# ivpml84079/Probabilistic-Self-Update-Line-Vector-Set-Based-Point-Cloud-Registration

Hardware: NVIDIA B200
Metric: registrations/s (higher is better)
Workload: dtype f64+f32

## Files before the change

probabilistic-self-update-line-vector-set-based-point-cloud-registration_b200/csrc/capi.cu:

```cuda
#include <cuda_runtime.h>

#include <cmath>
#include <cstring>
#include <new>
#include <string>
#include <vector>

#include "common.cuh"
#include "engine.cuh"

namespace psulvsb {

static thread_local std::string g_last_error;

void set_error(const std::string& msg) { g_last_error = msg; }
int fail(int code, const std::string& msg) {
  g_last_error = msg;
  return code;
}

int sm_count() {
  static int cached[64];
  int dev = 0;
  if (cudaGetDevice(&dev) != cudaSuccess || dev < 0 || dev >= 64) return 148;
// ... 18 lines not shown
  }
  return PSULVSB_OK;
}

namespace {

template <typename T>
struct DeviceJob {
  T* d = nullptr;
  cudaStream_t st;
  explicit DeviceJob(cudaStream_t s) : st(s) {}
  int put(const T& h) {
    PSU_CUDA(cudaMallocAsync((void**)&d, sizeof(T), st));
    PSU_CUDA(cudaMemcpyAsync(d, &h, sizeof(T), cudaMemcpyHostToDevice, st));
    return PSULVSB_OK;
  }
  ~DeviceJob() {
    if (d) cudaFreeAsync(d, st);
  }
};

}
}

using namespace psulvsb;

struct psulvsb_handle_s {
  EnginePool* pool;
  Comm* comm;
  int device;
};

extern "C" {

int psulvsb_version(void) { return PSULVSB_VERSION; }

const char* psulvsb_last_error(void) { return g_last_error.c_str(); }

void psulvsb_default_params(psulvsb_params_t* p) {
  if (!p) return;
  std::memset(p, 0, sizeof(*p));
  p->noise_bound = 0.01;
  p->cbar2 = 1;
  p->estimate_scaling = 1;
  p->rotation_max_iterations = 100;
  p->rotation_gnc_factor = 1.4;
  p->rotation_cost_threshold = 1e-6;
  p->inlier_selection_mode = 0;
  p->kcore_heuristic_threshold = 0.5;
  p->score_noise_bound = 0.01;
  p->inloop_noise_bound = 0.05;
  p->inloop_cbar2 = 1;
  p->inloop_max_iterations = 100;
  p->inloop_gnc_factor = 1.4;
  p->inloop_cost_threshold = 0.005;
  p->rotation_similar = 0.01;
  p->local_max_iter = 10;
  p->tpro_host = 0.99;
  p->tpro_local = 0.99;
  p->host_round_limit = 5;
  p->wallclock_cap_s = 60.0;
  p->self_update = 1;
  p->seed = 0;
}

int psulvsb_device_count(void) {
  int n = 0;
  if (cudaGetDeviceCount(&n) != cudaSuccess) {
    cudaGetLastError();
    return 0;
  }
  return n;
}

int psulvsb_create(psulvsb_handle_t* out, int device) {
  if (!out) return fail(PSULVSB_ERR_INVALID, "psulvsb_create: out is NULL");
  *out = nullptr;
  if (int rc = need_device()) return rc;
  psulvsb_handle_s* h = new (std::nothrow) psulvsb_handle_s();
  if (!h) return fail(PSULVSB_ERR_INTERNAL, "out of host memory");
  h->comm = nullptr;
  h->device = device;
  const int rc = pool_create(&h->pool, device);
  if (rc) {
    delete h;
    return rc;
  }
  *out = h;
  return PSULVSB_OK;
}

int psulvsb_destroy(psulvsb_handle_t h) {
  if (!h) return PSULVSB_OK;
  comm_destroy(h->comm);
  pool_destroy(h->pool);
  delete h;
  return PSULVSB_OK;
}

int psulvsb_solve(psulvsb_handle_t h, const psulvsb_params_t* params, const psulvsb_problem_t* problem,
                  psulvsb_solution_t* solution, psulvsb_trace_t* trace) {
  if (!h || !params || !problem || !solution) return fail(PSULVSB_ERR_INVALID, "psulvsb_solve: NULL argument");
  return pool_solve_one(h->pool, params, problem, solution, trace);
}

int psulvsb_solve_batch(psulvsb_handle_t h, const psulvsb_params_t* params, const psulvsb_problem_t* problems, int B,
                        const uint64_t* seeds, psulvsb_solution_t* solutions) {
  if (!h || !params || !problems || !solutions || B <= 0)
    return fail(PSULVSB_ERR_INVALID, "psulvsb_solve_batch: NULL argument or B <= 0");
  return pool_solve_batch(h->pool, params, problems, B, seeds, solutions);
}

int psulvsb_batch_submit(psulvsb_handle_t h, const psulvsb_params_t* params, const psulvsb_problem_t* problems, int B,
                         const uint64_t* seeds, psulvsb_solution_t* solutions, uint64_t* ticket) {
  if (!h || !params || !problems || !solutions || !ticket || B <= 0)
    return fail(PSULVSB_ERR_INVALID, "psulvsb_batch_submit: NULL argument or B <= 0");
  return pool_submit(h->pool, params, problems, B, seeds, solutions, ticket);
}

int psulvsb_batch_wait(psulvsb_handle_t h, uint64_t ticket) {
  if (!h) return fail(PSULVSB_ERR_INVALID, "psulvsb_batch_wait: NULL handle");
  return pool_wait(h->pool, ticket);
}

int psulvsb_batch_upload(psulvsb_handle_t h, const psulvsb_problem_t* problems, int B) {
  if (!h || !problems || B <= 0) return fail(PSULVSB_ERR_INVALID, "psulvsb_batch_upload: NULL argument or B <= 0");
  return pool_upload(h->pool, problems, B);
}

int psulvsb_batch_solve_resident(psulvsb_handle_t h, const psulvsb_params_t* params, const uint64_t* seeds,
                                 psulvsb_solution_t* solutions, int n_solutions) {
  if (!h || !params || !solutions) return fail(PSULVSB_ERR_INVALID, "psulvsb_batch_solve_resident: NULL argument");
  const int B = pool_batch_size(h->pool);
  if (B <= 0) return fail(PSULVSB_ERR_INVALID, "psulvsb_batch_solve_resident: nothing is resident (upload first)");
  if (n_solutions != B)
    return fail(PSULVSB_ERR_INVALID, "psulvsb_batch_solve_resident: " + std::to_string(n_solutions) +
                                         " solution slots for a resident batch of " + std::to_string(B));
  return pool_solve_resident(h->pool, params, seeds, solutions, nullptr);
}

int psulvsb_debug_set(const char* name, double value) {
  if (!name) return fail(PSULVSB_ERR_INVALID, "psulvsb_debug_set: NULL name");
  DebugKnobs& k = debug_knobs();
  const std::string n(name);
  if (n == "gnc_deep_margin") k.gnc_deep_margin = value;
  else if (n == "gnc_prefetch") k.gnc_prefetch = (int)value;
  else if (n == "gnc_cluster") k.gnc_cluster = (int)value;
  else if (n == "gnc_park_pct") k.gnc_park_pct = (int)value;
  else if (n == "gnc_cps") k.gnc_cps = (int)value;
  else if (n == "gnc_grid_lv") k.gnc_grid_lv = (int)value;
  else if (n == "sample_list_cap_test") k.sample_list_cap_test = (int)value;
  else if (n == "k1_variant") k.k1_variant = (int)value;
  else if (n == "upload_prof") k.upload_prof = (int)value;
  else if (n == "reset") k = DebugKnobs();
  else return fail(PSULVSB_ERR_INVALID, "psulvsb_debug_set: unknown switch " + n);
  return PSULVSB_OK;
}

int psulvsb_batch_resident_size(psulvsb_handle_t h) { return h ? pool_batch_size(h->pool) : 0; }

int psulvsb_set_batching(psulvsb_handle_t h, int chunk, int lanes) {
  if (!h) return fail(PSULVSB_ERR_INVALID, "psulvsb_set_batching: NULL handle");
  return pool_set_batching(h->pool, chunk, lanes);
}

int psulvsb_set_host_threads(psulvsb_handle_t h, int n) {
  if (!h) return fail(PSULVSB_ERR_INVALID, "psulvsb_set_host_threads: NULL handle");
  return pool_set_host_threads(h->pool, n);
}

long long psulvsb_launch_count(psulvsb_handle_t h) { return h ? pool_launch_count(h->pool) : 0; }
double psulvsb_last_device_ms(psulvsb_handle_t h) { return h ? pool_last_device_ms(h->pool) : 0.0; }
double psulvsb_last_stage_ms(psulvsb_handle_t h, int which) { return h ? pool_last_stage_ms(h->pool, which) : 0.0; }
int psulvsb_last_ticks(psulvsb_handle_t h) { return h ? pool_last_ticks(h->pool) : 0; }
int psulvsb_last_chunk_ticks(psulvsb_handle_t h, int* out, int cap) {
  if (!h || (cap > 0 && !out)) return 0;
  return pool_last_chunk_ticks(h->pool, out, cap);
}


int psulvsb_pack_points(void* stream, const double* d_pts, int n, const double center[3], void* d_out_float4) {
  if (int rc = need_device()) return rc;
  if (!d_pts || !d_out_float4 || n < 0) return fail(PSULVSB_ERR_INVALID, "psulvsb_pack_points: bad argument");
  return launch_pack_points((cudaStream_t)stream, d_pts, n, center, (float4*)d_out_float4);
}

int psulvsb_consistency_mask_rows(void* stream, const void* d_src_f4, const void* d_dst_f4, const double* d_src64,
                                  const double* d_dst64, int n, int row_begin, int row_end, double beta,
                                  double coord_bound, uint32_t* d_mask, int row_stride_words, uint32_t* d_row_counts,
                                  unsigned long long* d_border_count) {
  if (int rc = need_device()) return rc;
  if (!d_src_f4 || !d_dst_f4 || !d_src64 || !d_dst64 || !d_mask)
    return fail(PSULVSB_ERR_INVALID, "psulvsb_consistency_mask: NULL array");
  if (n < 1 || row_begin < 0 || row_end > n || row_begin > row_end)
    return fail(PSULVSB_ERR_INVALID, "psulvsb_consistency_mask: bad n / row range");
  if (row_stride_words < (n + 31) / 32)
    return fail(PSULVSB_ERR_CAPACITY, "psulvsb_consistency_mask: row_stride_words < ceil(n / 32)");
  if (!(beta >= 0.0) || !(coord_bound >= 0.0) || !std::isfinite(beta) || !std::isfinite(coord_bound))
    return fail(PSULVSB_ERR_INVALID, "psulvsb_consistency_mask: beta / coord_bound must be finite and >= 0");
  if (((uintptr_t)d_src_f4 & 15) || ((uintptr_t)d_dst_f4 & 15))
    return fail(PSULVSB_ERR_INVALID, "psulvsb_consistency_mask: float4 arrays must be 16-byte aligned");
  if (row_begin == row_end) return PSULVSB_OK;
  cudaStream_t st = (cudaStream_t)stream;
  float4* il = nullptr;
  const size_t nrec = il_records((size_t)n);
  PSU_CUDA(cudaMallocAsync((void**)&il, sizeof(float4) * 2 * nrec, st));
  struct IlFree {
    float4* p;
    cudaStream_t s;
    ~IlFree() { cudaFreeAsync(p, s); }
  } il_free{il, st};
  if (int rc = launch_interleave_points(st, (const float4*)d_src_f4, n, il)) return rc;
  if (int rc = launch_interleave_points(st, (const float4*)d_dst_f4, n, il + nrec)) return rc;
  K1Job j;
  std::memset(&j, 0, sizeof(j));
  j.src = il;
  j.dst = il + nrec;
  j.src64 = d_src64;
  j.dst64 = d_dst64;
  j.n = n;
  j.row_begin = row_begin;
  j.row_end = row_end;
  j.c = make_k1_consts(beta, coord_bound);
  j.mask = d_mask;
  j.stride = row_stride_words;
  j.row_counts = d_row_counts;
  j.border = d_border_count;
  j.active = 1;
  if (d_row_counts) PSU_CUDA(cudaMemsetAsync(d_row_counts + row_begin, 0, sizeof(uint32_t) * (size_t)(row_end - row_begin), st));
  PSU_CUDA(cudaMemsetAsync(d_mask + (size_t)row_begin * row_stride_words, 0,
                           sizeof(uint32_t) * (size_t)(row_end - row_begin) * row_stride_words, st));
  DeviceJob<K1Job> dj(st);
  if (int rc = dj.put(j)) return rc;
  return launch_consistency_mask(st, dj.d, 1, n, row_end - row_begin, (row_stride_words & 7) == 0);
}

int psulvsb_consistency_mask(void* stream, const void* d_src_f4, const void* d_dst_f4, const double* d_src64,
                             const double* d_dst64, int n, double beta, double coord_bound, uint32_t* d_mask,
                             int row_stride_words, uint32_t* d_row_counts, unsigned long long* d_border_count) {
  return psulvsb_consistency_mask_rows(stream, d_src_f4, d_dst_f4, d_src64, d_dst64, n, 0, n, beta, coord_bound, d_mask,
                                       row_stride_words, d_row_counts, d_border_count);
}

int psulvsb_mask_symmetrize(void* stream, uint32_t* d_mask, int n, int row_stride_words) {
  if (int rc = need_device()) return rc;
  if (!d_mask || n < 1 || row_stride_words < (n + 31) / 32)
    return fail(PSULVSB_ERR_INVALID, "psulvsb_mask_symmetrize: bad argument");
  return launch_symmetrize((cudaStream_t)stream, d_mask, n, row_stride_words);
}

int psulvsb_compact_edges(void* stream, const uint32_t* d_mask, int n, int row_stride_words,
                          const uint32_t* d_row_counts, unsigned long long* d_row_offsets, void* d_edges_uint2,
                          unsigned long long edge_capacity, unsigned long long* d_n_edges) {
  if (int rc = need_device()) return rc;
  if (!d_mask || !d_row_counts || !d_row_offsets || n < 1 || row_stride_words < (n + 31) / 32)
    return fail(PSULVSB_ERR_INVALID, "psulvsb_compact_edges: bad argument");
  cudaStream_t st = (cudaStream_t)stream;
  CompactJob j;
  std::memset(&j, 0, sizeof(j));
  j.mask = d_mask;
  j.n = n;
  j.stride = row_stride_words;
  j.row_counts = d_row_counts;
  j.offsets = d_row_offsets;
  j.edges = (uint2*)d_edges_uint2;
  j.cap = edge_capacity;
  j.n_edges = d_n_edges;
  j.active = 1;
  DeviceJob<CompactJob> dj(st);
  if (int rc = dj.put(j)) return rc;
  return launch_compact_edges(st, dj.d, 1, n, true, d_edges_uint2 != nullptr);
}

int psulvsb_ratio_reduced_set(void* stream, const double* d_src64, const double* d_dst64, int n, uint32_t* d_pair_bin,
                              void* d_edges_uint2, unsigned long long edge_capacity, unsigned long long* n_edges,
                              double* max_scale, unsigned int peak[2]) {
  if (!d_src64 || !d_dst64 || !n_edges || n < 2)
    return fail(PSULVSB_ERR_INVALID, "psulvsb_ratio_reduced_set: NULL array / n_edges, or n < 2");
  if (int rc = need_device()) return rc;
  cudaStream_t st = (cudaStream_t)stream;
  const size_t L = (size_t)n * (size_t)(n - 1) / 2;
  size_t off = 0;
  auto take = [&](size_t bytes) {
    const size_t o = (off + 15) & ~(size_t)15;
    off = o + bytes;
    return o;
  };
  const size_t o_bins = d_pair_bin ? 0 : take(sizeof(uint32_t) * L);
  const size_t o_rmax = take(sizeof(double) * (size_t)n), o_bpi = take(sizeof(unsigned long long) * RATIO_MAX_GROWTHS),
               o_bps = take(sizeof(double) * RATIO_MAX_GROWTHS), o_bpn = take(sizeof(unsigned int)),
               o_fs = take(sizeof(double)), o_bad = take(sizeof(int)), o_peak = take(4 * sizeof(unsigned int)),
               o_cc = take(sizeof(unsigned int) * 3 * (size_t)n),
               o_co = take(sizeof(unsigned long long) * (3 * (size_t)n + 1)), o_ne = take(sizeof(unsigned long long));
  struct Scratch {
    char* p = nullptr;
    void* hist = nullptr;
    cudaStream_t s;
    ~Scratch() {
      if (p) cudaFreeAsync(p, s);
      if (hist) cudaFreeAsync(hist, s);
    }
  } scr;
  scr.s = st;
  PSU_CUDA(cudaMallocAsync((void**)&scr.p, off, st));
  std::vector<RatioJob> rj(1);
  RatioJob& j = rj[0];
  std::memset(&j, 0, sizeof(j));
  j.src64 = d_src64;
  j.dst64 = d_dst64;
  j.n = n;
  j.pair_bin = d_pair_bin ? d_pair_bin : reinterpret_cast<uint32_t*>(scr.p + o_bins);
  j.row_max = reinterpret_cast<double*>(scr.p + o_rmax);
  j.bp_idx = reinterpret_cast<unsigned long long*>(scr.p + o_bpi);
  j.bp_scale = reinterpret_cast<double*>(scr.p + o_bps);
  j.bp_n = reinterpret_cast<unsigned int*>(scr.p + o_bpn);
  j.final_scale = reinterpret_cast<double*>(scr.p + o_fs);
  j.bad = reinterpret_cast<int*>(scr.p + o_bad);
  j.peak = reinterpret_cast<unsigned int*>(scr.p + o_peak);
  j.class_counts = reinterpret_cast<unsigned int*>(scr.p + o_cc);
  j.class_offsets = reinterpret_cast<unsigned long long*>(scr.p + o_co);
  j.n_edges = reinterpret_cast<unsigned long long*>(scr.p + o_ne);
  j.active = 1;
  DeviceJob<RatioJob> dj(st);
  if (int rc = dj.put(j)) return rc;
  auto arena = [&](size_t bytes) -> void* {
    const cudaError_t e = cudaMallocAsync(&scr.hist, bytes, st);
    if (e == cudaSuccess) return scr.hist;
    scr.hist = nullptr;
    fail(PSULVSB_ERR_CUDA, std::string("psulvsb_ratio_reduced_set: histogram allocation: ") + cudaGetErrorString(e));
    return nullptr;
  };
  if (int rc = ratio_count(st, rj, dj.d, n, arena, nullptr, nullptr)) return rc;
  unsigned long long ne = 0;
  double fs = 0.0;
  unsigned int pk[2] = {0u, 0u};
  PSU_CUDA(cudaMemcpyAsync(&ne, j.n_edges, sizeof(ne), cudaMemcpyDeviceToHost, st));
  PSU_CUDA(cudaMemcpyAsync(&fs, j.final_scale, sizeof(fs), cudaMemcpyDeviceToHost, st));
  PSU_CUDA(cudaMemcpyAsync(pk, j.peak, sizeof(pk), cudaMemcpyDeviceToHost, st));
  PSU_CUDA(cudaStreamSynchronize(st));
  *n_edges = ne;
  if (max_scale) *max_scale = fs;
  if (peak) {
    peak[0] = pk[0];
    peak[1] = pk[1];
  }
  if (!d_edges_uint2) return PSULVSB_OK;
  if (ne > edge_capacity)
    return fail(PSULVSB_ERR_CAPACITY, "psulvsb_ratio_reduced_set: " + std::to_string(ne) + " edges, capacity " +
                                          std::to_string(edge_capacity));
  j.edges = (uint2*)d_edges_uint2;
  j.cap = edge_capacity;
  if (int rc = ratio_emit(st, rj, dj.d, n)) return rc;
  PSU_CUDA(cudaStreamSynchronize(st));
  return PSULVSB_OK;
}

unsigned long long psulvsb_sample_default_max_draws(unsigned long long n, unsigned long long count) {
  return sample_default_max_draws(n, count);
}

unsigned long long psulvsb_sample_workspace_bytes(unsigned long long n, unsigned long long count,
                                                  unsigned long long max_draws) {
  if (max_draws == 0) max_draws = sample_default_max_draws(n, count);
  return ((sample_table_words(n, max_draws) * sizeof(uint32_t) + 15) & ~15ull) +
         sample_chunk_slots(max_draws) * sizeof(unsigned long long) + 16 +
         sample_list_counters() * sizeof(unsigned int) + sample_list_entries(n, max_draws) * sizeof(uint32_t);
}

int psulvsb_sample(void* stream, uint64_t seed, uint32_t domain, uint32_t event, unsigned long long n,
                   unsigned long long count, unsigned long long max_draws, uint32_t* d_out, void* d_work,
                   unsigned long long* d_status) {
  if (int rc = need_device()) return rc;
  if (!d_out || !d_work || !d_status) return fail(PSULVSB_ERR_INVALID, "psulvsb_sample: NULL array");
  if (n == 0 || count > n) return fail(PSULVSB_ERR_INVALID, "psulvsb_sample: need 0 < n and count <= n");
  if (n >= 0x7FFFFFFFull) return fail(PSULVSB_ERR_UNSUPPORTED, "psulvsb_sample: n must fit the 31-bit draws");
  if (max_draws == 0) max_draws = sample_default_max_draws(n, count);
  if (max_draws >= 0xFFFFFFFFull) return fail(PSULVSB_ERR_UNSUPPORTED, "psulvsb_sample: max_draws must be < 2^32 - 1");
  cudaStream_t st = (cudaStream_t)stream;
  const size_t first_bytes = (sample_table_words(n, max_draws) * sizeof(uint32_t) + 15) & ~15ull;
  const size_t slots = sample_chunk_slots(max_draws);
  PSU_CUDA(cudaMemsetAsync(d_work, 0, first_bytes, st));
  PSU_CUDA(cudaMemsetAsync((char*)d_work + first_bytes + slots * sizeof(unsigned long long), 0, 16, st));
  PSU_CUDA(cudaMemsetAsync(d_status, 0, sizeof(unsigned long long), st));
  if (count == 0) return PSULVSB_OK;
  SampleJob j;
  std::memset(&j, 0, sizeof(j));
  j.seed = seed;
  j.domain = domain;
  j.event = event;
  j.n = n;
  j.count = count;
  j.max_draws = max_draws;
  j.first = (uint32_t*)d_work;
  j.chunk_prefix = (unsigned long long*)((char*)d_work + first_bytes);
  j.ticket = (unsigned int*)((char*)d_work + first_bytes + slots * sizeof(unsigned long long));
  {
    char* p = (char*)d_work + first_bytes + slots * sizeof(unsigned long long) + 16;
    j.bcount = (unsigned int*)p;
    PSU_CUDA(cudaMemsetAsync(p, 0, sample_list_counters() * sizeof(unsigned int), st));
    j.blist_cap = sample_list_entries(n, max_draws);
    j.blist = j.blist_cap ? (uint32_t*)(p + sample_list_counters() * sizeof(unsigned int)) : nullptr;
  }
  j.out = d_out;
  j.status = d_status;
  j.active = 1;
  DeviceJob<SampleJob> dj(st);
  if (int rc = dj.put(j)) return rc;
  return launch_sample(st, dj.d, 1, max_draws, n);
}

int psulvsb_philox_fill(void* stream, uint64_t seed, uint32_t domain, uint32_t event, unsigned long long first_k,
                        unsigned long long count, uint32_t* d_out_rand31) {
  if (int rc = need_device()) return rc;
  if (!d_out_rand31 && count) return fail(PSULVSB_ERR_INVALID, "psulvsb_philox_fill: NULL output");
  return launch_philox_fill((cudaStream_t)stream, seed, domain, event, first_k, count, d_out_rand31);
}

int psulvsb_gnc_tls_rotation(void* stream, const double* d_src64, const double* d_dst64, const void* d_edges_uint2,
                             unsigned long long K, double inv_scale, double noise_bound, int max_iterations,
                             double gnc_factor, double cost_threshold, const double* d_R_init, double* d_weights,
                             double* d_R, uint8_t* d_inliers, int* d_info, double* d_cost) {
  if (int rc = need_device()) return rc;
  if (!d_src64 || !d_dst64 || (!d_edges_uint2 && K) || !d_R || (!d_weights && K))
    return fail(PSULVSB_ERR_INVALID, "psulvsb_gnc_tls_rotation: NULL array");
  if (max_iterations < 0) return fail(PSULVSB_ERR_INVALID, "psulvsb_gnc_tls_rotation: max_iterations < 0");
  if (K >= 0x7FFFFFF0ull) return fail(PSULVSB_ERR_UNSUPPORTED, "psulvsb_gnc_tls_rotation: K must fit 31 bits");
  cudaStream_t st = (cudaStream_t)stream;
  GncJob j;
  std::memset(&j, 0, sizeof(j));
  j.src = d_src64;
  j.dst = d_dst64;
  j.edges = (const uint2*)d_edges_uint2;
  j.K = K;
  j.inv_scale = inv_scale;
  j.noise_bound = noise_bound;
  j.gnc_factor = gnc_factor;
  j.cost_threshold = cost_threshold;
  j.max_iterations = max_iterations;
  j.use_init = d_R_init ? 1 : 0;
  if (d_R_init) PSU_CUDA(cudaMemcpyAsync(j.R_init, d_R_init, sizeof(double) * 9, cudaMemcpyDeviceToHost, st));
  if (d_R_init) PSU_CUDA(cudaStreamSynchronize(st));
  j.weights = d_weights;
  j.lv = nullptr;
  j.lv_cap = 0;
  j.R_out = d_R;
  j.inliers = d_inliers;
  j.point_flags = nullptr;
  j.n_points = 0;
  j.info = d_info;
  j.cost = d_cost;
  j.active = 1;
  DeviceJob<GncJob> dj(st);
  if (int rc = dj.put(j)) return rc;
  int cap = (int)((K + 7) / 8) + 32;
  cap = (cap + 31) & ~31;
  return launch_gnc_tls(st, dj.d, 1, cap, 8);
}

int psulvsb_gnc_tls_rotation_batch(void* stream, const double* d_src64, const double* d_dst64, int n_points,
                                   const void* d_edges_uint2, unsigned long long K, int n_jobs, double noise_bound,
                                   int max_iterations, double gnc_factor, double cost_threshold, int cluster,
                                   double* d_weights, double* d_lv, unsigned long long lv_cap, uint32_t* d_perm,
                                   double* d_R, uint8_t* d_inliers, int* d_info, long long* d_prof) {
  if (int rc = need_device()) return rc;
  if (!d_src64 || !d_dst64 || !d_edges_uint2 || !d_R || !d_weights || n_jobs < 1 || K < 1)
    return fail(PSULVSB_ERR_INVALID, "psulvsb_gnc_tls_rotation_batch: bad argument");
  if (K >= 0x7FFFFFF0ull) return fail(PSULVSB_ERR_UNSUPPORTED, "psulvsb_gnc_tls_rotation_batch: K must fit 31 bits");
  cudaStream_t st = (cudaStream_t)stream;
  std::vector<GncJob> jobs((size_t)n_jobs);
  for (int b = 0; b < n_jobs; ++b) {
    GncJob& j = jobs[(size_t)b];
    std::memset(&j, 0, sizeof(j));
    j.src = d_src64;
    j.dst = d_dst64;
    j.edges = (const uint2*)d_edges_uint2 + (size_t)b * K;
    j.K = K;
    j.inv_scale = 1.0;
    j.noise_bound = noise_bound;
    j.gnc_factor = gnc_factor;
    j.cost_threshold = cost_threshold;
    j.max_iterations = max_iterations;
    j.weights = d_weights + (size_t)b * K;
    j.lv = d_lv ? d_lv + (size_t)b * 6 * lv_cap : nullptr;
    j.lv_cap = d_lv ? lv_cap : 0;
    j.perm = (d_lv && d_perm) ? d_perm + (size_t)b * 2 * lv_cap : nullptr;
    j.R_out = d_R + (size_t)b * 9;
    j.inliers = d_inliers ? d_inliers + (size_t)b * K : nullptr;
    j.n_points = n_points;
    j.info = d_info ? d_info + (size_t)b * 4 : nullptr;
    j.prof = d_prof ? d_prof + (size_t)b * 8 : nullptr;
    j.active = 1;
  }
  struct AsyncJobs {
    GncJob* d = nullptr;
    double* red = nullptr;
    unsigned int* bar = nullptr;
    cudaStream_t st;
    explicit AsyncJobs(cudaStream_t s) : st(s) {}
    ~AsyncJobs() {
      if (d) cudaFreeAsync(d, st);
      if (red) cudaFreeAsync(red, st);
      if (bar) cudaFreeAsync(bar, st);
    }
  } dj(st);
  const bool grid_mode = cluster > 8;
// ... 180 lines not shown
```

probabilistic-self-update-line-vector-set-based-point-cloud-registration_b200/csrc/common.cuh:

```cuda
#pragma once

#include <cuda_runtime.h>
#include <stdint.h>

#include <cstdio>
#include <string>

#include "../../include/psulvsb.h"

namespace psulvsb {

void set_error(const std::string& msg);
int fail(int code, const std::string& msg);

#define PSU_CUDA(call)                                                                              \
  do {                                                                                              \
    cudaError_t e__ = (call);                                                                       \
    if (e__ != cudaSuccess) {                                                                       \
      return ::psulvsb::fail(PSULVSB_ERR_CUDA, std::string(#call) + ": " + cudaGetErrorString(e__)); \
    }                                                                                               \
  } while (0)

#define PSU_CHECK_LAUNCH(name)                                                                      \
  do {                                                                                              \
    cudaError_t e__ = cudaGetLastError();                                                           \
    if (e__ != cudaSuccess) {                                                                       \
      return ::psulvsb::fail(PSULVSB_ERR_CUDA, std::string(name) + " launch: " + cudaGetErrorString(e__)); \
    }                                                                                               \
  } while (0)

int need_device();

int sm_count();

struct DebugKnobs {
  double gnc_deep_margin = 0.0;
  int gnc_cluster = 0;
  int gnc_prefetch = -1;
  int gnc_grid_lv = 0;
  int gnc_cps = 0;
  int gnc_park_pct = 0;
  int sample_list_cap_test = 0;
  int k1_variant = 0;
  int upload_prof = 0;
};
DebugKnobs& debug_knobs();

inline unsigned long long ceil_div_ull(unsigned long long a, unsigned long long b) { return (a + b - 1) / b; }
inline size_t translation_sort_doubles(int n_points) {
  size_t m = 1;
  while (m < (size_t)n_points + 1) m <<= 1;
  return m;
}

struct Philox4 {
  uint32_t w[4];
};

__host__ __device__ __forceinline__ uint32_t mulhi32(uint32_t a, uint32_t b) {
#ifdef __CUDA_ARCH__
  return __umulhi(a, b);
#else
  return (uint32_t)(((uint64_t)a * b) >> 32);
#endif
}

__host__ __device__ __forceinline__ Philox4 philox4x32_10(uint64_t seed, uint32_t domain, uint32_t event,
                                                          uint64_t block) {
  uint32_t c0 = (uint32_t)block, c1 = (uint32_t)(block >> 32), c2 = event, c3 = domain;
  uint32_t k0 = (uint32_t)seed, k1 = (uint32_t)(seed >> 32);
#pragma unroll
  for (int r = 0; r < 10; ++r) {
    const uint32_t hi0 = mulhi32(0xD2511F53u, c0), lo0 = 0xD2511F53u * c0;
    const uint32_t hi1 = mulhi32(0xCD9E8D57u, c2), lo1 = 0xCD9E8D57u * c2;
    const uint32_t n0 = hi1 ^ c1 ^ k0, n2 = hi0 ^ c3 ^ k1;
    c0 = n0;
    c1 = lo1;
    c2 = n2;
    c3 = lo0;
    k0 += 0x9E3779B9u;
    k1 += 0xBB67AE85u;
  }
  Philox4 o;
  o.w[0] = c0;
  o.w[1] = c1;
  o.w[2] = c2;
  o.w[3] = c3;
  return o;
}

__host__ __device__ __forceinline__ uint32_t philox_rand31(uint64_t seed, uint32_t domain, uint32_t event,
                                                           uint64_t k) {
  Philox4 o = philox4x32_10(seed, domain, event, k >> 2);
  return o.w[k & 3] >> 1;
}

__host__ __device__ __forceinline__ double philox_uniform01(uint64_t seed, uint32_t domain, uint32_t event,
                                                            uint64_t k) {
  Philox4 o = philox4x32_10(seed, domain, event, k);
  return ((double)(o.w[0] >> 5) * 67108864.0 + (double)(o.w[1] >> 6)) / 9007199254740992.0;
}

__device__ __forceinline__ double dmul(double a, double b) { return __dmul_rn(a, b); }
__device__ __forceinline__ double dadd(double a, double b) { return __dadd_rn(a, b); }
__device__ __forceinline__ double dsub(double a, double b) { return __dsub_rn(a, b); }

__device__ __forceinline__ double sqnorm3(double x, double y, double z) {
  return dadd(dadd(dmul(x, x), dmul(y, y)), dmul(z, z));
}

__device__ __forceinline__ float4 pack_point(double x, double y, double z) {
  const float xf = (float)x, yf = (float)y, zf = (float)z;
  const double n2 = (double)xf * (double)xf + (double)yf * (double)yf + (double)zf * (double)zf;
  return make_float4(xf, yf, zf, (float)n2);
}

__host__ __device__ inline size_t il_records(size_t n) { return (n + 1) & ~(size_t)1; }
__device__ __forceinline__ void il_store(float4* __restrict__ il, int i, const float4 p) {
  float* f = reinterpret_cast<float*>(il + (i & ~1)) + (i & 1);
  f[0] = p.x;
  f[2] = p.y;
  f[4] = p.z;
  f[6] = p.w;
}
__device__ __forceinline__ float4 il_load(const float4* __restrict__ il, int i) {
  const float* f = reinterpret_cast<const float*>(il + (i & ~1)) + (i & 1);
  return make_float4(f[0], f[2], f[4], f[6]);
}

#ifdef __CUDACC__
__device__ __forceinline__ uint32_t smem_u32(const void* p) { return (uint32_t)__cvta_generic_to_shared(p); }

__device__ __forceinline__ void mbar_init(uint64_t* bar, uint32_t count) {
  asm volatile("mbarrier.init.shared::cta.b64 [%0], %1;" ::"r"(smem_u32(bar)), "r"(count));
}
__device__ __forceinline__ void mbar_expect_tx(uint64_t* bar, uint32_t bytes) {
  asm volatile("mbarrier.arrive.expect_tx.shared::cta.b64 _, [%0], %1;" ::"r"(smem_u32(bar)), "r"(bytes) : "memory");
}
__device__ __forceinline__ bool mbar_try_wait(uint64_t* bar, uint32_t parity) {
  uint32_t ok;
  asm volatile(
      "{\n"
      ".reg .pred p;\n"
      "mbarrier.try_wait.parity.shared::cta.b64 p, [%1], %2;\n"
      "selp.u32 %0, 1, 0, p;\n"
      "}\n"
      : "=r"(ok)
      : "r"(smem_u32(bar)), "r"(parity)
      : "memory");
  return ok != 0;
}
__device__ __forceinline__ void mbar_wait(uint64_t* bar, uint32_t parity) {
  while (!mbar_try_wait(bar, parity)) {
  }
}
__device__ __forceinline__ void mbar_arrive(uint64_t* bar) {
  asm volatile("mbarrier.arrive.shared::cta.b64 _, [%0];" ::"r"(smem_u32(bar)) : "memory");
}
__device__ __forceinline__ void tma_load_1d(void* smem_dst, const void* gmem_src, uint32_t bytes, uint64_t* bar) {
  asm volatile("cp.async.bulk.shared::cluster.global.mbarrier::complete_tx::bytes [%0], [%1], %2, [%3];" ::"r"(
                   smem_u32(smem_dst)),
               "l"(gmem_src), "r"(bytes), "r"(smem_u32(bar))
               : "memory");
}

__device__ __forceinline__ float2 fma2(const float2 a, const float2 b, const float2 c) {
  unsigned long long ra, rb, rc, rd;
  asm("mov.b64 %0, {%1, %2};" : "=l"(ra) : "f"(a.x), "f"(a.y));
  asm("mov.b64 %0, {%1, %2};" : "=l"(rb) : "f"(b.x), "f"(b.y));
  asm("mov.b64 %0, {%1, %2};" : "=l"(rc) : "f"(c.x), "f"(c.y));
  asm("fma.rn.f32x2 %0, %1, %2, %3;" : "=l"(rd) : "l"(ra), "l"(rb), "l"(rc));
  float2 d;
  asm("mov.b64 {%0, %1}, %2;" : "=f"(d.x), "=f"(d.y) : "l"(rd));
  return d;
}
__device__ __forceinline__ float2 add2(const float2 a, const float2 b) {
  unsigned long long ra, rb, rd;
  asm("mov.b64 %0, {%1, %2};" : "=l"(ra) : "f"(a.x), "f"(a.y));
  asm("mov.b64 %0, {%1, %2};" : "=l"(rb) : "f"(b.x), "f"(b.y));
  asm("add.rn.f32x2 %0, %1, %2;" : "=l"(rd) : "l"(ra), "l"(rb));
  float2 d;
  asm("mov.b64 {%0, %1}, %2;" : "=f"(d.x), "=f"(d.y) : "l"(rd));
  return d;
}
__device__ __forceinline__ float2 bc2(const float x) { return make_float2(x, x); }
#endif

struct Mat3d {
  double m[3][3];
};

__device__ __forceinline__ double warp_sum(double v) {
#pragma unroll
  for (int o = 16; o > 0; o >>= 1) v += __shfl_xor_sync(0xffffffffu, v, o);
  return v;
}
__device__ __forceinline__ double warp_max(double v) {
// ... 12 lines not shown
```

probabilistic-self-update-line-vector-set-based-point-cloud-registration_b200/csrc/engine.cu:

```cuda
#include <cuda_runtime.h>
#include <sched.h>

#include <algorithm>
#include <atomic>
#include <chrono>
#if defined(__SSE2__)
#include <emmintrin.h>
#endif
#include <cmath>
#include <cstdlib>
#include <cstring>
#include <condition_variable>
#include <deque>
#include <functional>
#include <map>
#include <memory>
#include <mutex>
#include <string>
#include <thread>
#include <utility>
#include <vector>

#include "common.cuh"
#include "engine.cuh"
// ... 493 lines not shown
      m.rj = bm.take<RatioJob>((size_t)B);
      m.bad = bm.take<int>((size_t)B);
      m.fscale = bm.take<double>((size_t)B);
      m.cq = bm.take<CliqueJob>((size_t)B);
      if (pass == 0) {
        if (int rc = d_misc.ensure(bm.off)) return rc;
        bm.base = reinterpret_cast<char*>(d_misc.p);
      }
    }
  }
  const double* in_dbl = reinterpret_cast<const double*>(d_in_dbl.p);
  const int* in_int = reinterpret_cast<const int*>(d_in_int.p);
  int maxC = 0, maxM = 0;
  {
    Bump bw, bk;
    for (int pass = 0; pass < 2; ++pass) {
      bw.off = 0;
      bk.off = 0;
      for (int b = 0; b < B; ++b) {
        const ProbLayout& L = lay[(size_t)(b0 + b)];
        JobCtl& J = jobs[(size_t)b];
        std::memset(&J, 0, sizeof(J));
        J.C0 = L.C0;
        J.M = L.M;
        J.Ccap = L.Ccap;
        J.src0 = in_dbl + L.in_dbl;
        J.dst0 = J.src0 + 3 * (size_t)L.C0;
        J.ori_src = L.alias_ori ? J.src0 : J.src0 + 6 * (size_t)L.C0;
        J.ori_dst = L.alias_ori ? J.dst0 : J.ori_src + 3 * (size_t)L.M;
        J.keep_mask0 = in_int + L.in_int;
        J.reduce_map0 = J.keep_mask0 + L.M;
        J.src = bw.take<double>((size_t)3 * L.Ccap);
        J.dst = bw.take<double>((size_t)3 * L.Ccap);
        J.pts8 = bw.take<double>((size_t)8 * L.Ccap);
        J.residual_history = bw.take<double>((size_t)L.M);
        J.xs = bw.take<double>((size_t)3 * (L.Ccap + 1));
        J.xs_sorted = bw.take<double>(translation_sort_doubles(L.Ccap));
        J.keep_mask = bw.take<int>((size_t)L.M);
        J.reduce_map = bw.take<int>((size_t)L.M);
        J.inlier_counter = bw.take<int>((size_t)L.M);
        J.new_corr = bw.take<int>((size_t)L.M);
        J.inlier_history = bw.take<int>((size_t)L.M);
        J.final_inliers = bw.take<int>((size_t)L.M);
        J.hs_bits = bw.take<uint32_t>(2 * (((size_t)L.M + 31) / 32) + 2);
        J.inlier_map = bw.take<int>((size_t)L.Ccap);
        J.idx = bw.take<int>((size_t)L.Ccap);
        J.adj_stride = (L.Ccap + 31) / 32;
        J.adj = params->inlier_selection_mode != 3 ? bw.take<uint32_t>(clique_scratch_words(L.Ccap)) : nullptr;
        J.clique_flags = bw.take<uint8_t>((size_t)L.Ccap);
        J.sampled_flags = bw.take<uint8_t>((size_t)L.Ccap);
        J.rot_flags = bw.take<uint8_t>((size_t)L.Ccap);
        J.local_trace = bw.take<psulvsb_local_trace_t>((size_t)local_cap);
        J.host_trace = bw.take<psulvsb_host_trace_t>((size_t)host_cap);
        J.local_trace_cap = local_cap;
        J.host_trace_cap = host_cap;
        J.estimate_scaling = ratio ? 1 : 0;
        J.seed = seeds ? seeds[b] : params->seed + (uint64_t)b;
        const float a = 1 + (((float)L.C0) / (long)L.M);
        J.tau = 2 * params->score_noise_bound * a;
        float4* sf = bw.take<float4>(il_records((size_t)L.C0));
        float4* df = bw.take<float4>(il_records((size_t)L.C0));
        K1Job& K = k1[(size_t)b];
        std::memset(&K, 0, sizeof(K));
        K.src = sf;
        K.dst = df;
        K.src64 = J.src0;
        K.dst64 = J.dst0;
        K.n = L.C0;
        K.row_begin = sharded ? row_b : 0;
        K.row_end = sharded ? row_e : L.C0;
        K.c = make_k1_consts(2.0 * params->noise_bound * std::sqrt(params->cbar2), L.coord_bound);
        K.mask = ratio ? nullptr : bk.take<uint32_t>((size_t)L.C0 * L.stride);
        K.stride = L.stride;
        K.row_counts = bk.take<uint32_t>((size_t)L.C0);
        if (ratio) {
          RatioJob& Rj = rj[(size_t)b];
          std::memset(&Rj, 0, sizeof(Rj));
          Rj.src64 = J.src0;
          Rj.dst64 = J.dst0;
          Rj.n = L.C0;
          Rj.pair_bin = bk.take<uint32_t>((size_t)L.C0 * (size_t)(L.C0 - 1) / 2 + 1);
          Rj.row_max = bk.take<double>((size_t)L.C0);
          Rj.bp_idx = bk.take<unsigned long long>(RATIO_MAX_GROWTHS);
          Rj.bp_scale = bk.take<double>(RATIO_MAX_GROWTHS);
          Rj.bp_n = bk.take<unsigned int>(1);
          Rj.final_scale = m.fscale + b;
          Rj.peak = bk.take<unsigned int>(4);
          Rj.class_counts = bk.take<unsigned int>((size_t)3 * L.C0);
          Rj.class_offsets = bk.take<unsigned long long>((size_t)3 * L.C0 + 1);
          Rj.n_edges = m.n_edges + b;
          Rj.bad = m.bad + b;
          Rj.active = 1;
        }
        K.border = m.border + b;
        K.active = 1;
        CompactJob& Cj = cj[(size_t)b];
        std::memset(&Cj, 0, sizeof(Cj));
        Cj.mask = K.mask;
        Cj.n = L.C0;
        Cj.stride = L.stride;
        Cj.row_counts = K.row_counts;
        Cj.offsets = bk.take<unsigned long long>((size_t)L.C0 + 1);
        Cj.n_edges = m.n_edges + b;
        Cj.active = 1;
        PackJob& p0 = pj[(size_t)2 * b];
        PackJob& p1 = pj[(size_t)2 * b + 1];
        p0.pts = J.src0;
        p0.out = sf;
        p0.n = L.C0;
        p0.zero = K.row_counts;
        p1.zero = nullptr;
        p1.pts = J.dst0;
        p1.out = df;
        p1.n = L.C0;
        for (int r = 0; r < 3; ++r) {
          p0.c[r] = L.csrc[r];
          p1.c[r] = L.cdst[r];
        }
        maxC = L.C0 > maxC ? L.C0 : maxC;
        maxM = L.M > maxM ? L.M : maxM;
      }
      if (pass == 0) {
        if (int rc = d_work.ensure(bw.off)) return rc;
        if (int rc = d_mask.ensure(bk.off)) return rc;
        bw.base = reinterpret_cast<char*>(d_work.p);
        bk.base = reinterpret_cast<char*>(d_mask.p);
      }
    }
    PSU_CUDA(cudaEventRecord(ev_begin, st));
  }
  PSU_CUDA(cudaMemsetAsync(m.border, 0, sizeof(unsigned long long) * (size_t)B, st));
  PSU_CUDA(cudaMemsetAsync(m.n_done, 0, sizeof(int) * 4, st));
  PSU_CUDA(cudaMemcpyAsync(m.k1, k1.data(), sizeof(K1Job) * (size_t)B, cudaMemcpyHostToDevice, st));
  PSU_CUDA(cudaMemcpyAsync(m.cj, cj.data(), sizeof(CompactJob) * (size_t)B, cudaMemcpyHostToDevice, st));
  PSU_CUDA(cudaMemcpyAsync(m.pj, pj.data(), sizeof(PackJob) * (size_t)2 * B, cudaMemcpyHostToDevice, st));

  if (ratio) {
    if (int rc = ratio_count(st, rj, m.rj, maxC, [&](size_t bytes) -> void* { return d_hist.ensure(bytes) ? nullptr : d_hist.p; },
                             ev_m0, ev_m1))
      return rc;
    launches += 8;
  } else {
    {
      dim3 grid((unsigned)((maxC + 255) / 256), (unsigned)(2 * B));
      engine_pack_kernel<<<grid, 256, 0, st>>>(m.pj);
      PSU_CHECK_LAUNCH("engine_pack_kernel");
      ++launches;
    }
    PSU_CUDA(cudaEventRecord(ev_m0, st));
    if (!sharded || row_e > row_b)
      if (int rc = launch_consistency_mask(st, m.k1, B, maxC, sharded ? row_e - row_b : maxC, true)) return rc;
    PSU_CUDA(cudaEventRecord(ev_m1, st));
    ++launches;
    if (int rc = launch_compact_edges(st, m.cj, B, maxC, true, false)) return rc;
    ++launches;
  }
  if (int rc = h_small.ensure((sizeof(unsigned long long) + sizeof(int)) * (size_t)B + 64 + 66 * sizeof(unsigned long long)))
    return rc;
  unsigned long long* h_nedges = reinterpret_cast<unsigned long long*>(h_small.p);
  volatile int* h_done = reinterpret_cast<volatile int*>(reinterpret_cast<char*>(h_small.p) + sizeof(unsigned long long) * (size_t)B);
  unsigned long long* h_counts = reinterpret_cast<unsigned long long*>(
      reinterpret_cast<char*>(h_small.p) + align_up((sizeof(unsigned long long) + sizeof(int)) * (size_t)B + 16, 16));
  std::vector<unsigned long long> shard_off;
  if (sharded) {
    if (int rc = comm_allgather_u64(comm, st, m.n_edges, m.counts_all)) return rc;
    PSU_CUDA(cudaMemcpyAsync(h_counts, m.counts_all, sizeof(unsigned long long) * (size_t)comm_world(comm),
                             cudaMemcpyDeviceToHost, st));
    PSU_CUDA(cudaStreamSynchronize(st));
    shard_off.assign((size_t)comm_world(comm) + 1, 0ull);
    for (int r = 0; r < comm_world(comm); ++r) shard_off[(size_t)r + 1] = shard_off[(size_t)r] + h_counts[r];
    h_nedges[0] = shard_off.back();
    PSU_CUDA(cudaMemcpyAsync(m.n_edges, h_nedges, sizeof(unsigned long long), cudaMemcpyHostToDevice, st));
  } else {
    PSU_CUDA(cudaMemcpyAsync(h_nedges, m.n_edges, sizeof(unsigned long long) * (size_t)B, cudaMemcpyDeviceToHost, st));
    PSU_CUDA(cudaStreamSynchronize(st));
  }

  const int grid_ctas_max = sm_count() / (B > 0 ? B : 1);
  unsigned long long max_cap = 0, max_nred = 0;
  {
    Bump be;
    for (int pass = 0; pass < 2; ++pass) {
      be.off = 0;
      for (int b = 0; b < B; ++b) {
        JobCtl& J = jobs[(size_t)b];
        unsigned long long cap = h_nedges[b] + reserve[(size_t)(b0 + b)];
        if (cap < 64) cap = 64;
        J.edge_cap = cap;
        J.edges = be.take<uint2>((size_t)cap);
        J.first_words = sample_table_words(cap, sample_default_max_draws(cap, cap));
        J.first = be.take<uint32_t>((size_t)J.first_words);
        J.draws_cap = (cap + 3) & ~3ull;
        J.draws = be.take<uint32_t>((size_t)J.draws_cap);
        J.chunk_prefix = be.take<unsigned long long>((size_t)sample_chunk_slots(sample_default_max_draws(cap, cap)));
        J.ticket = be.take<unsigned int>(4);
        J.blist_cap = sample_list_entries(cap, cap) ? sample_list_entries(cap, cap) : 0ull;
        J.blist = J.blist_cap ? be.take<uint32_t>((size_t)J.blist_cap) : nullptr;
        J.bcount = be.take<unsigned int>((size_t)sample_list_counters());
        J.vbits = be.take<uint32_t>((size_t)((cap + 31) / 32 + 32));
        J.L_sampled = be.take<uint32_t>((size_t)cap);
        J.basic_idx = be.take<uint32_t>((size_t)cap);
        J.basic_edges = be.take<uint2>((size_t)cap);
        J.weights = be.take<double>((size_t)cap);
        J.lv_cap = cap / 6 + 64;
        J.lv = be.take<double>((size_t)6 * J.lv_cap);
        J.gnc_perm = be.take<uint32_t>((size_t)2 * J.lv_cap);
        if (grid_ctas_max >= 16) {
          J.gnc_grid_red = be.take<double>((size_t)grid_ctas_max * GNC_GRID_RED_DOUBLES);
          J.gnc_grid_bar = be.take<unsigned int>(4);
        }
        J.pruned_edges = ratio ? be.take<uint2>((size_t)cap) : nullptr;
        if (ratio) {
          rj[(size_t)b].edges = J.edges;
          rj[(size_t)b].cap = cap;
        }
        cj[(size_t)b].edges = J.edges + (sharded && be.base ? shard_off[(size_t)comm_rank(comm)] : 0ull);
        cj[(size_t)b].cap = cap - (sharded ? shard_off[(size_t)comm_rank(comm)] : 0ull);
        max_cap = cap > max_cap ? cap : max_cap;
        max_nred = h_nedges[b] > max_nred ? h_nedges[b] : max_nred;
      }
      if (pass == 0) {
        if (int rc = d_edge.ensure(be.off)) return rc;
        be.base = reinterpret_cast<char*>(d_edge.p);
      }
    }
  }
  if (max_cap >= 0x7FFFFFF0ull) return fail(PSULVSB_ERR_UNSUPPORTED, "reduced set exceeds the 31-bit sample / line-vector indices");
  PSU_CUDA(cudaMemcpyAsync(m.jobs, jobs.data(), sizeof(JobCtl) * (size_t)B, cudaMemcpyHostToDevice, st));
  if (ratio) {
    if (int rc = ratio_emit(st, rj, m.rj, maxC)) return rc;
  } else {
    PSU_CUDA(cudaMemcpyAsync(m.cj, cj.data(), sizeof(CompactJob) * (size_t)B, cudaMemcpyHostToDevice, st));
    if (int rc = launch_compact_edges(st, m.cj, B, maxC, false, true)) return rc;
    if (sharded) {
      std::vector<unsigned long long> off32(shard_off);
      for (auto& o : off32) o *= 2ull;
      if (int rc = comm_allgatherv_inplace_u32(comm, st, reinterpret_cast<uint32_t*>(jobs[0].edges), off32.data())) return rc;
    }
  }
  ++launches;

  EngineParams P;
  P.caller = SubParams{params->noise_bound, params->cbar2, params->rotation_max_iterations, params->rotation_gnc_factor,
                       params->rotation_cost_threshold};
  P.inloop = SubParams{params->inloop_noise_bound, params->inloop_cbar2, params->inloop_max_iterations,
                       params->inloop_gnc_factor, params->inloop_cost_threshold};
  P.pr_noise = 2 * params->score_noise_bound;
  P.score_sigma = params->score_noise_bound;
  P.rotation_similar = params->rotation_similar;
  P.local_max_iter = params->local_max_iter;
  P.tpro_host = params->tpro_host;
  P.tpro_local = params->tpro_local;
  P.host_round_limit = params->host_round_limit;
  P.wallclock_cap_s = params->wallclock_cap_s;
  P.self_update = params->self_update;
  P.inlier_selection_mode = params->inlier_selection_mode;
  P.max_local_iters = 4096;
  P.split_host_scoring = (maxM >= 32768) ? 1 : 0;
  P.sampler_counters = (int)sample_list_counters();
  {
    unsigned long long sig = 1469598103934665603ull;
    auto mix = [&](unsigned long long v) { sig = (sig ^ v) * 1099511628211ull; };
    for (int b = 0; b < B; ++b) {
      const JobCtl& J = jobs[(size_t)b];
      mix((unsigned long long)(uintptr_t)J.first);
      mix(J.first_words);
      mix((unsigned long long)(uintptr_t)J.vbits);
      mix(J.edge_cap);
    }
    P.zero_sampler_scratch = (sampler_scratch_sig == sig && sampler_scratch_clean) ? 0 : 1;
    sampler_scratch_sig = sig;
    sampler_scratch_clean = false;
  }
  {
    int init_y = (int)(((long long)sm_count() * 2 + B - 1) / B);
    const int by_size = (std::max(maxM, maxC) + 4 * kCtlThreads - 1) / (4 * kCtlThreads);
    if (init_y > by_size) init_y = by_size;
    if (init_y < 1) init_y = 1;
    engine_init_kernel<<<dim3((unsigned)B, (unsigned)init_y), kCtlThreads, 0, st>>>(m.jobs, m.sl, m.sb, m.gj, m.cq, m.n_edges, P,
                                                                                    m.n_done);
  }
  PSU_CHECK_LAUNCH("engine_init_kernel");
  ++launches;
  PSU_CUDA(cudaEventRecord(ev_k1, st));

  int n_running = B;
  int max_ccap = 0;
  for (int b = 0; b < B; ++b) max_ccap = lay[(size_t)(b0 + b)].Ccap > max_ccap ? lay[(size_t)(b0 + b)].Ccap : max_ccap;
  const unsigned long long draws_bound = sample_default_max_draws(max_cap, max_cap / 8 + 1);
  int ticks = 0;
  double gnc_ms = 0.0;
  gnc_iv.clear();
  const int max_ticks = P.max_local_iters + P.host_round_limit + 8;
  bool round_start_pending = true;
  bool clique_pending = false;
  while (true) {
    const double elapsed =
        std::chrono::duration_cast<std::chrono::microseconds>(std::chrono::steady_clock::now() - t_begin).count() / 1e6;
    if (round_start_pending) {
      engine_round_start_kernel<<<B, kCtlThreads, 0, st>>>(m.jobs, m.sl, m.sb, m.gj, m.cq, P, m.n_done);
      PSU_CHECK_LAUNCH("engine_round_start_kernel");
      if (int rc = launch_sample(st, m.sl, B, draws_bound, max_cap, true)) return rc;
      launches += 5;
    }
    if (int rc = launch_sample(st, m.sb, B, draws_bound, max_cap)) return rc;
    if (ratio) {
      engine_scale_kernel<<<B, kCtlThreads, 0, st>>>(m.jobs, m.gj, m.cq, P);
      PSU_CHECK_LAUNCH("engine_scale_kernel");
      ++launches;
    }
    if (clique_pending) {
      int maxCcap = 0;
      for (int b = 0; b < B; ++b) maxCcap = lay[(size_t)(b0 + b)].Ccap > maxCcap ? lay[(size_t)(b0 + b)].Ccap : maxCcap;
      if (int rc = launch_max_clique(st, m.cq, B, maxCcap, (maxCcap + 31) / 32, max_cap, params->inlier_selection_mode == 0))
        return rc;
      launches += 8;
    }
    PSU_CUDA(cudaEventRecord(ev_g0, st));
    int gnc_cluster = gnc_cluster_for(n_running);
    if (gnc_cluster == 8 && grid_ctas_max >= 16) {
      const long long k_est = (long long)(0.03 * (double)max_nred);
      const int lv_per_cta = debug_knobs().gnc_grid_lv > 0 ? debug_knobs().gnc_grid_lv : 4096;
      const long long g = std::min<long long>(grid_ctas_max, k_est / lv_per_cta);
      if (g >= 16) gnc_cluster = (int)g;
    }
    int gnc_cap = (int)((0.03 * (double)max_nred) / (double)gnc_cluster) + 64;
    gnc_cap = (gnc_cap + 31) & ~31;
    if (gnc_cap > gnc_default_capacity()) gnc_cap = gnc_default_capacity();
    if (int rc = launch_gnc_tls(st, m.gj, B, gnc_cap, gnc_cluster, n_running)) return rc;
    PSU_CUDA(cudaEventRecord(ev_g1, st));
    engine_local_control_kernel<<<B, kCtlThreads, 0, st>>>(m.jobs, m.sl, m.sb, m.gj, m.cq, P, elapsed, m.n_done);
    PSU_CHECK_LAUNCH("engine_local_control_kernel");
    launches += 5;
    if (P.split_host_scoring) {
      engine_host_score_kernel<<<dim3((unsigned)((maxM + kCtlThreads - 1) / kCtlThreads), (unsigned)B), kCtlThreads, 0, st>>>(
          m.jobs, P);
      PSU_CHECK_LAUNCH("engine_host_score_kernel");
      engine_host_finish_kernel<<<B, kCtlThreads, 0, st>>>(m.jobs, m.sb, m.gj, m.cq, P, elapsed, m.n_done);
      PSU_CHECK_LAUNCH("engine_host_finish_kernel");
      launches += 2;
    }
    ++ticks;
    PSU_CUDA(cudaMemcpyAsync((void*)h_done, m.n_done, 3 * sizeof(int), cudaMemcpyDeviceToHost, st));
    PSU_CUDA(cudaStreamSynchronize(st));
    {
      float g = 0.f;
      if (cudaEventElapsedTime(&g, ev_g0, ev_g1) == cudaSuccess) gnc_ms += g;
      float a = 0.f;
      if (origin && cudaEventElapsedTime(&a, origin, ev_g0) == cudaSuccess) gnc_iv.emplace_back(a, a + g);
    }
    if (debug_knobs().upload_prof) {
      const double now = std::chrono::duration_cast<std::chrono::microseconds>(std::chrono::steady_clock::now() - t_begin).count() / 1e3;
      std::fprintf(stderr, "tick %d: ends %.3f ms after the solve began; done %d of %d, waiting for a round start %d, clique %d\n",
                   ticks, now, h_done[0], B, h_done[1], h_done[2]);
    }
    if (h_done[0] >= B) break;
    n_running = B - h_done[0];
    round_start_pending = h_done[1] > 0;
    clique_pending = h_done[2] > 0 && params->inlier_selection_mode != 3;
    if (ticks >= max_ticks) return fail(PSULVSB_ERR_INTERNAL, "engine did not converge within the tick limit");
  }
  last_ticks = ticks;
  PSU_CUDA(cudaEventRecord(ev_loop, st));
  engine_refine_kernel<<<B, kCtlThreads, 0, st>>>(m.jobs, m.sols, m.border);
  PSU_CHECK_LAUNCH("engine_refine_kernel");
  ++launches;
  PSU_CUDA(cudaMemcpyAsync(solutions, m.sols, sizeof(psulvsb_solution_t) * (size_t)B, cudaMemcpyDeviceToHost, st));
  PSU_CUDA(cudaEventRecord(ev_end, st));
  PSU_CUDA(cudaStreamSynchronize(st));
  sampler_scratch_clean = true;
  float ms = 0.f;
  cudaEventElapsedTime(&ms, ev_begin, ev_end);
  last_ms = ms;
  cudaEventElapsedTime(&ms, ev_begin, ev_k1);
  stage_ms[0] = ms;
  cudaEventElapsedTime(&ms, ev_k1, ev_loop);
  stage_ms[1] = ms;
  cudaEventElapsedTime(&ms, ev_loop, ev_end);
  stage_ms[4] = ms;
  cudaEventElapsedTime(&ms, ev_m0, ev_m1);
  stage_ms[2] = ms;
  stage_ms[3] = gnc_ms;
  if (origin) {
    cudaEventElapsedTime(&off_begin, origin, ev_begin);
    cudaEventElapsedTime(&off_end, origin, ev_end);
    cudaEventElapsedTime(&off_m0, origin, ev_m0);
    cudaEventElapsedTime(&off_m1, origin, ev_m1);
  }

  if (trace_first) {
    JobCtl j0;
    PSU_CUDA(cudaMemcpy(&j0, m.jobs, sizeof(JobCtl), cudaMemcpyDeviceToHost));
    trace_first->local_n = 0;
    trace_first->host_n = 0;
    if (trace_first->local && trace_first->local_cap > 0) {
      const int n = j0.n_local_trace < trace_first->local_cap ? j0.n_local_trace : trace_first->local_cap;
      if (n > 0)
        PSU_CUDA(cudaMemcpy(trace_first->local, j0.local_trace, sizeof(psulvsb_local_trace_t) * (size_t)n,
                            cudaMemcpyDeviceToHost));
      trace_first->local_n = n;
    }
    if (trace_first->host && trace_first->host_cap > 0) {
      const int n = j0.n_host_trace < trace_first->host_cap ? j0.n_host_trace : trace_first->host_cap;
      if (n > 0)
        PSU_CUDA(cudaMemcpy(trace_first->host, j0.host_trace, sizeof(psulvsb_host_trace_t) * (size_t)n,
                            cudaMemcpyDeviceToHost));
      trace_first->host_n = n;
    }
    if (trace_first->final_inliers)
      PSU_CUDA(cudaMemcpy(trace_first->final_inliers, j0.final_inliers, sizeof(int) * (size_t)j0.M, cudaMemcpyDeviceToHost));
    if (trace_first->inlier_counter)
      PSU_CUDA(cudaMemcpy(trace_first->inlier_counter, j0.inlier_counter, sizeof(int) * (size_t)j0.M, cudaMemcpyDeviceToHost));
    if (trace_first->reduce_map_out)
      PSU_CUDA(cudaMemcpy(trace_first->reduce_map_out, j0.reduce_map, sizeof(int) * (size_t)j0.M, cudaMemcpyDeviceToHost));
  }
  return PSULVSB_OK;
}

namespace {
double union_ms(std::vector<std::pair<float, float>>& iv) {
  if (iv.empty()) return 0.0;
  std::sort(iv.begin(), iv.end());
  double total = 0.0;
  float lo = iv[0].first, hi = iv[0].second;
  for (size_t i = 1; i < iv.size(); ++i) {
    if (iv[i].first > hi) {
      total += hi - lo;
      lo = iv[i].first;
      hi = iv[i].second;
    } else if (iv[i].second > hi) {
      hi = iv[i].second;
    }
  }
  return total + (hi - lo);
}
}

namespace {
int available_cpus() {
  cpu_set_t set;
  CPU_ZERO(&set);
  if (sched_getaffinity(0, sizeof(set), &set) == 0) {
    const int n = CPU_COUNT(&set);
    if (n > 0) return n;
  }
  const int hw = (int)std::thread::hardware_concurrency();
  return hw > 0 ? hw : 1;
}
}

class EnginePool {
 public:
  int device = 0;
  int chunk = 0;
  int lanes = 0;
  int host_threads = 0;
  std::vector<Engine*> eng;
  cudaEvent_t origin = nullptr;
// ... 461 lines not shown
```

probabilistic-self-update-line-vector-set-based-point-cloud-registration_b200/csrc/engine.cuh:

```cuda
#pragma once

#include <cuda_runtime.h>
#include <math.h>
#include <stdint.h>

#include <functional>
#include <vector>

#include "common.cuh"

namespace psulvsb {

struct K1Consts {
  float half_bias;
  float two_beta2;
  float r0;
  float kappa;
  float w_thr;
  double beta;
  float beta4;
  float t_fast;
};
K1Consts make_k1_consts(double beta, double coord_bound);

struct K1Job {
  const float4* src;
  const float4* dst;
  const double* src64;
  const double* dst64;
  int n, row_begin, row_end;
  K1Consts c;
  uint32_t* mask;
  int stride;
  uint32_t* row_counts;
  unsigned long long* border;
  int active;
};

struct CompactJob {
  const uint32_t* mask;
  int n, stride;
  const uint32_t* row_counts;
  unsigned long long* offsets;
  uint2* edges;
  unsigned long long cap;
  unsigned long long* n_edges;
  int active;
};

constexpr double RATIO_MAX_SCALE = 2.0e6;
constexpr int RATIO_MAX_GROWTHS = 8;
struct RatioJob {
  const double* src64;
  const double* dst64;
  int n;
  uint32_t* pair_bin;
  unsigned int* hist;
  unsigned long long* last;
  double* row_max;
  unsigned long long* bp_idx;
  double* bp_scale;
  unsigned int* bp_n;
  double* final_scale;
  unsigned int* peak;
  unsigned int* class_counts;
  unsigned long long* class_offsets;
  unsigned long long* n_edges;
  uint2* edges;
  unsigned long long cap;
  int* bad;
  int active;
};

struct SampleJob {
  uint64_t seed;
  uint32_t domain, event;
  unsigned long long n, count, max_draws;
  uint32_t* first;
  unsigned long long* chunk_prefix;
  unsigned int* ticket;
  uint32_t* draws;
  unsigned long long draws_cap;
  uint32_t* blist;
  unsigned long long blist_cap;
  unsigned int* bcount;
  uint32_t* out;
  unsigned long long* status;
  int identity;
  int post;
  const uint2* edges;
  const uint32_t* via;
  uint2* gathered;
  const double* pts8;
  double* lv_out;
  unsigned long long lv_cap;
  uint8_t* flags;
  uint32_t* vbits;
  int n_points;
  int active;
};

struct GncJob {
  const double* src;
  const double* dst;
  const double* pts8;
  const uint2* edges;
  unsigned long long K;
  double inv_scale;
  double noise_bound;
  double gnc_factor;
  double cost_threshold;
  int max_iterations;
  int use_init;
  double R_init[9];
  double* weights;
  double* lv;
  unsigned long long lv_cap;
  uint32_t* perm;
  int lv_ready;
  double* R_out;
  uint8_t* inliers;
  uint8_t* point_flags;
  int n_points;
  int* info;
  double* cost;
  long long* prof;
  double* grid_red;
  unsigned int* grid_bar;
  int active;
};
constexpr int GNC_GRID_RED_DOUBLES = 2 * 16;

struct CliqueJob {
  const uint2* edges;
  unsigned long long n_edges;
  const double* src;
  const double* dst;
  double beta;
  int filter;
  int n_vertices;
  uint32_t* adj;
  int stride;
  uint8_t* flags;
  int* size;
  int* proven;
  int active;
};
inline size_t clique_scratch_words(int n_vertices) {
  return (((size_t)n_vertices * (size_t)((n_vertices + 31) / 32) + 3) & ~(size_t)3) + 8;
}
int launch_max_clique(cudaStream_t st, const CliqueJob* d_jobs, int n_jobs, int max_vertices, int max_stride,
                      unsigned long long max_edges, bool exact);

int launch_knn_normals(cudaStream_t st, const double* pts, int n, int k, const double* viewpoint, double* normals);

int launch_pack_points(cudaStream_t st, const double* pts, int n, const double center[3], float4* out);
int launch_interleave_points(cudaStream_t st, const float4* in, int n, float4* out);
int launch_consistency_mask(cudaStream_t st, const K1Job* d_jobs, int n_jobs, int max_n, int max_rows, bool row_sectors);
int launch_symmetrize(cudaStream_t st, uint32_t* mask, int n, int stride);
int launch_compact_edges(cudaStream_t st, const CompactJob* d_jobs, int n_jobs, int max_n, bool scan, bool emit);
int ratio_count(cudaStream_t st, std::vector<RatioJob>& rj, RatioJob* d_rj, int max_n,
                const std::function<void*(size_t)>& hist_arena, cudaEvent_t ev0, cudaEvent_t ev1);
int ratio_emit(cudaStream_t st, const std::vector<RatioJob>& rj, RatioJob* d_rj, int max_n);

__host__ __device__ inline unsigned long long sample_max_draws_formula(unsigned long long n,
                                                                       unsigned long long count) {
  if (n == 0 || count == 0) return 0;
  if (count > n) count = n;
  double e;
  if (count == n) {
    e = (double)n * (log((double)n) + 0.5772156649 + 10.0);
  } else {
    const double f = (double)count / (double)n;
    const double mean = -(double)n * log1p(-f);
    e = mean * 1.02 + 8.0 * sqrt(mean + 1.0) + 64.0;
  }
  unsigned long long m = (unsigned long long)e + 8;
  m = (m + 3) & ~3ull;
  if (m > 0xFFFFFFF0ull) m = 0xFFFFFFF0ull;
  return m;
}
unsigned long long sample_default_max_draws(unsigned long long n, unsigned long long count);
unsigned long long sample_chunk_slots(unsigned long long max_draws);
unsigned long long sample_list_entries(unsigned long long n, unsigned long long max_draws);
unsigned long long sample_list_counters();
unsigned long long sample_table_words(unsigned long long n, unsigned long long max_draws);
int launch_sample(cudaStream_t st, const SampleJob* d_jobs, int n_jobs, unsigned long long max_draws_bound,
                  unsigned long long n_bound, bool flag_pass = false);
int launch_philox_fill(cudaStream_t st, uint64_t seed, uint32_t domain, uint32_t event, unsigned long long first_k,
                       unsigned long long count, uint32_t* out);

int gnc_default_capacity();
int gnc_cluster_for(int n_jobs);
int launch_gnc_tls(cudaStream_t st, const GncJob* d_jobs, int n_jobs, int cap_per_cta, int cluster, int n_active = 0);
int launch_kabsch_batch(cudaStream_t st, const double* src, const double* dst, const uint2* edges,
                        const uint32_t* sets, int k, unsigned long long n_hyp, double* R, double* t);

int launch_tls_translation(cudaStream_t st, const double* src, const double* dst, const uint8_t* flags, int n,
                           double scale, const double* R, double noise, const double* last_best, double* t_out,
                           int* n_points);
int launch_score_one(cudaStream_t st, const double* src, const double* dst, int n, double scale, const double* R,
                     const double* t, double tau, uint8_t* inliers, double* residuals, int* count);
int launch_score_batch(cudaStream_t st, const float4* src, const float4* dst, const double* src64, const double* dst64,
                       int n, const double* hyp, unsigned long long n_hyp, unsigned long long hyp_begin, double scale,
                       double tau, double coord_bound, const double* csrc, const double* cdst, uint32_t* counts,
                       unsigned long long* best, unsigned long long* border);

struct Comm;
int comm_unique_id(void* out128);
int comm_create(Comm** out, int device, int rank, int world, const void* id128);
void comm_destroy(Comm* c);
int comm_rank(const Comm* c);
int comm_world(const Comm* c);
int comm_allreduce_sum_u32(Comm* c, cudaStream_t st, uint32_t* d_inout, size_t n);
int comm_allreduce_max_u64(Comm* c, cudaStream_t st, unsigned long long* d_inout, size_t n);
int comm_allgather_u64(Comm* c, cudaStream_t st, const unsigned long long* d_send, unsigned long long* d_recv);
int comm_allgatherv_inplace_u32(Comm* c, cudaStream_t st, uint32_t* base, const unsigned long long* offsets);
void triangular_row_range(int n, int rank, int world, int* begin, int* end);

class EnginePool;
int pool_create(EnginePool** out, int device);
void pool_destroy(EnginePool* p);
int pool_set_batching(EnginePool* p, int chunk, int lanes);
int pool_set_host_threads(EnginePool* p, int n);
int pool_solve_one(EnginePool* p, const psulvsb_params_t* params, const psulvsb_problem_t* problem,
                   psulvsb_solution_t* solution, psulvsb_trace_t* trace);
int pool_solve_batch(EnginePool* p, const psulvsb_params_t* params, const psulvsb_problem_t* problems, int B,
                     const uint64_t* seeds, psulvsb_solution_t* solutions);
int pool_submit(EnginePool* p, const psulvsb_params_t* params, const psulvsb_problem_t* problems, int B,
                const uint64_t* seeds, psulvsb_solution_t* solutions, uint64_t* ticket);
int pool_wait(EnginePool* p, uint64_t ticket);
int pool_upload(EnginePool* p, const psulvsb_problem_t* problems, int B);
int pool_solve_sharded(EnginePool* p, Comm* comm, const psulvsb_params_t* params, const psulvsb_problem_t* problem,
                       psulvsb_solution_t* solution, psulvsb_trace_t* trace);
int pool_solve_resident(EnginePool* p, const psulvsb_params_t* params, const uint64_t* seeds,
                        psulvsb_solution_t* solutions, psulvsb_trace_t* trace_first);
int pool_batch_size(const EnginePool* p);
int pool_last_ticks(const EnginePool* p);
int pool_last_chunk_ticks(const EnginePool* p, int* out, int cap);
long long pool_launch_count(const EnginePool* p);
double pool_last_device_ms(const EnginePool* p);
double pool_last_stage_ms(const EnginePool* p, int which);

}
```

probabilistic-self-update-line-vector-set-based-point-cloud-registration_b200/csrc/engine_kernels.cu:

```cuda
#include <cuda_runtime.h>

#include "common.cuh"
#include "engine.cuh"
#include "engine_kernels.cuh"
#include "engine_state.cuh"
#include "solve_dev.cuh"
#include "svd3.cuh"

namespace psulvsb {

static_assert(kCtlThreads == BLK, "control kernels assume BLK threads");

namespace {

__device__ __constant__ double kLRate[4] = {0.1, 0.2, 0.5, 1.0};
__device__ __constant__ double kBRate[4] = {0.3, 0.3, 0.3, 1.0};

__device__ __forceinline__ void xform_identity(Xform& x) {
  x.s = 1.0;
#pragma unroll
  for (int i = 0; i < 9; ++i) x.R[i] = (i % 4 == 0) ? 1.0 : 0.0;
  x.t[0] = x.t[1] = x.t[2] = 0.0;
}

// ... 40 lines not shown
  const double scale = 1.0;
  g.src = J.src;
  g.dst = J.dst;
  g.edges = J.basic_edges;
  g.K = (unsigned long long)J.basic_choose;
  g.inv_scale = 1.0 / scale;
  g.noise_bound = J.cur.noise_bound * (2.0 / scale);
  g.gnc_factor = J.cur.gnc_factor;
  g.cost_threshold = J.cur.cost_threshold;
  g.max_iterations = J.cur.max_iterations;
  g.use_init = J.first_time ? 0 : 1;
#pragma unroll
  for (int c = 0; c < 3; ++c)
#pragma unroll
    for (int r = 0; r < 3; ++r) g.R_init[c * 3 + r] = J.last_best.R[r * 3 + c];
  g.weights = J.weights;
  g.lv = J.lv;
  g.lv_cap = J.lv_cap;
  g.perm = J.gnc_perm;
  g.grid_red = J.gnc_grid_red;
  g.grid_bar = J.gnc_grid_bar;
  g.pts8 = J.pts8;
  g.lv_ready = (J.estimate_scaling || sb.identity) ? 0 : 1;
  g.R_out = J.R_gnc;
  g.inliers = nullptr;
  g.point_flags = J.rot_flags;
  g.n_points = J.C;
  g.info = J.gnc_info;
  g.prof = nullptr;
  g.cost = &J.gnc_cost;
  g.active = 1;
  q.active = (J.rate_idx == 3 && P.inlier_selection_mode != 3) ? 1 : 0;
  q.edges = J.basic_edges;
  q.n_edges = (unsigned long long)J.basic_choose;
  q.src = J.src;
  q.dst = J.dst;
  q.beta = 2.0 * J.cur.noise_bound * sqrt(J.cur.cbar2);
  q.filter = 1;
  q.n_vertices = J.C;
  q.adj = J.adj;
  q.stride = J.adj_stride;
  q.flags = J.clique_flags;
  q.size = &J.clique_size;
  q.proven = &J.clique_proven;
}

__device__ int count_flagged(BlockScratch* s, const JobCtl& J, const Xform& X) {
  int cnt = 0, dummy = 0;
  for (int j = threadIdx.x; j < J.C; j += BLK)
    if (J.sampled_flags[j] && residual_ref(J.src + 3 * (size_t)j, J.dst + 3 * (size_t)j, X.s, X.R, X.t) <= J.tau) ++cnt;
  block_sum_int2(s, cnt, dummy);
  return cnt;
}

}

__global__ void __launch_bounds__(BLK)
    engine_init_kernel(JobCtl* __restrict__ jobs, SampleJob* __restrict__ sl, SampleJob* __restrict__ sb,
                       GncJob* __restrict__ gj, CliqueJob* __restrict__ cq,
                       const unsigned long long* __restrict__ n_edges, EngineParams P,
                       int* __restrict__ n_done) {
  JobCtl& J = jobs[blockIdx.x];
  const int tid = blockIdx.y * BLK + threadIdx.x;
  const int stride = gridDim.y * BLK;
  for (int i = tid; i < 3 * J.C0; i += stride) {
    J.src[i] = J.src0[i];
    J.dst[i] = J.dst0[i];
  }
  for (int i = tid; i < J.C0; i += stride) {
#pragma unroll
    for (int r = 0; r < 3; ++r) {
      J.pts8[8 * (size_t)i + r] = J.src0[3 * (size_t)i + r];
      J.pts8[8 * (size_t)i + 3 + r] = J.dst0[3 * (size_t)i + r];
    }
    J.pts8[8 * (size_t)i + 6] = 0.0;
    J.pts8[8 * (size_t)i + 7] = 0.0;
  }
  for (int j = tid; j < J.M; j += stride) {
    J.keep_mask[j] = J.keep_mask0[j];
    J.reduce_map[j] = J.reduce_map0[j];
    J.inlier_counter[j] = 0;
    J.new_corr[j] = 0;
    J.inlier_history[j] = -1;
    J.final_inliers[j] = 0;
    J.residual_history[j] = 0.0;
  }
  if (P.zero_sampler_scratch)
    for (unsigned long long i = tid; i < J.first_words; i += stride) J.first[i] = 0u;
  for (int i = tid; i < P.sampler_counters; i += stride) J.bcount[i] = 0u;
  if (P.zero_sampler_scratch)
    for (unsigned long long i = tid; i < (J.edge_cap + 31) / 32 + 32; i += stride) J.vbits[i] = 0u;
  if (tid == 0) {
    *J.ticket = 0u;
    J.C = J.C0;
    J.n_red0 = n_edges[blockIdx.x];
    J.n_red = J.n_red0;
    J.n_ls = 0;
    J.n_sampled_pts = 0;
    J.basic_choose = 0;
    J.phase = PHASE_ROUND_START;
    J.status = PSULVSB_OK;
    J.rounds_left = P.host_round_limit;
    J.host_round = 0;
    J.local_iter_global = 0;
    J.host_scorings = 0;
    J.escalations = 0;
    J.first_time = 1;
    J.sampled_first_time = 1;
    J.inloop = 0;
    J.longholi = 0;
    J.rate_idx = 0;
    J.local_r = 0;
    J.host_r = 0;
    J.best_sampled_cnt = 0;
    J.best_host_cnt = 0;
    J.pro_local = 0.0;
    J.pro_host = 0.0;
    J.pro_host_not_over = 1;
    J.scale_noise = 0.0;
    J.translation_noise = 0.0;
    xform_identity(J.sol);
    xform_identity(J.best_sampled);
    xform_identity(J.best_host);
    xform_identity(J.last_best);
    J.new_corr_count = 0;
    J.inlier_map_size = 0;
    J.scale_calls = 0;
    J.n_pruned = 0;
    J.cur_scale = 1.0;
    J.sample_status[0] = J.sample_status[1] = 1ull;
    J.n_local_trace = 0;
    J.n_host_trace = 0;
    J.valid = 0;
    J.refined = 0;
    sl[blockIdx.x].active = 0;
    sb[blockIdx.x].active = 0;
    gj[blockIdx.x].active = 0;
    cq[blockIdx.x].active = 0;
    J.clique_size = 0;
    J.aborted = 0;
    if (J.n_red0 > J.edge_cap) {
      J.status = PSULVSB_ERR_CAPACITY;
      J.phase = PHASE_DONE;
      atomicAdd(n_done, 1);
    } else if (J.n_red0 == 0) {
      J.phase = PHASE_DONE;
      atomicAdd(n_done, 1);
    } else {
      atomicAdd(n_done + 1, 1);
    }
  }
}

__global__ void __launch_bounds__(BLK)
    engine_round_start_kernel(JobCtl* __restrict__ jobs, SampleJob* __restrict__ sl, SampleJob* __restrict__ sb,
                              GncJob* __restrict__ gj, CliqueJob* __restrict__ cq, EngineParams P,
                              int* __restrict__ n_done) {
  JobCtl& J = jobs[blockIdx.x];
  SampleJob& L = sl[blockIdx.x];
  const int tid = threadIdx.x;
  if (J.phase != PHASE_ROUND_START) {
    if (tid == 0) {
      L.active = 0;
      if (J.phase == PHASE_DONE) {
        sb[blockIdx.x].active = 0;
        gj[blockIdx.x].active = 0;
        cq[blockIdx.x].active = 0;
      }
    }
    return;
  }
  __shared__ int ok_s;
  if (tid == 0) atomicSub(n_done + 1, 1);
  const int nnew = (P.self_update ? J.new_corr_count : 0);
  const int m0 = J.inlier_map_size;
  const int C = J.C;
  if (tid == 0) {
    const unsigned long long extra = (unsigned long long)nnew * (unsigned long long)m0 +
                                     (unsigned long long)nnew * (unsigned long long)(nnew > 0 ? nnew - 1 : 0) / 2ull;
    ok_s = (J.n_red + extra <= J.edge_cap && C + nnew <= J.Ccap) ? 1 : 0;
  }
  __syncthreads();
  if (!ok_s) {
    if (tid == 0) {
      J.status = PSULVSB_ERR_CAPACITY;
      J.phase = PHASE_DONE;
      L.active = 0;
      sb[blockIdx.x].active = 0;
      gj[blockIdx.x].active = 0;
      atomicAdd(n_done, 1);
    }
    return;
  }
  if (nnew > 0) {
    for (int i = tid; i < nnew; i += BLK) {
      const int o = J.new_corr[i];
#pragma unroll
      for (int r = 0; r < 3; ++r) {
        J.src[3 * (size_t)(C + i) + r] = J.ori_src[3 * (size_t)o + r];
        J.dst[3 * (size_t)(C + i) + r] = J.ori_dst[3 * (size_t)o + r];
        J.pts8[8 * (size_t)(C + i) + r] = J.ori_src[3 * (size_t)o + r];
        J.pts8[8 * (size_t)(C + i) + 3 + r] = J.ori_dst[3 * (size_t)o + r];
      }
      J.pts8[8 * (size_t)(C + i) + 6] = 0.0;
      J.pts8[8 * (size_t)(C + i) + 7] = 0.0;
      J.keep_mask[o] = 1;
      J.reduce_map[o] = C + i;
    }
    const unsigned long long base = J.n_red;
    for (int i = 0; i < nnew; ++i) {
      const unsigned long long off = base + (unsigned long long)i * m0 + (unsigned long long)i * (i > 0 ? i - 1 : 0) / 2ull;
      const int cnt = m0 + i;
      for (int j = tid; j < cnt; j += BLK) {
        const int other = (j < m0) ? J.inlier_map[j] : (C + (j - m0));
        J.edges[off + j] = make_uint2((unsigned)(C + i), (unsigned)other);
      }
    }
  }
  __syncthreads();
  if (tid == 0) {
    if (nnew > 0) {
      J.n_red += (unsigned long long)nnew * m0 + (unsigned long long)nnew * (nnew - 1) / 2ull;
      J.C = C + nnew;
    }
    J.rounds_left -= 1;
    J.new_corr_count = 0;
    J.inlier_map_size = 0;
    J.sampled_first_time = 1;
    J.best_sampled_cnt = 0;
    J.local_r = 0;
    J.pro_local = 0.0;
    const double l_rate = kLRate[J.rate_idx];
    unsigned long long n_ls = (unsigned long long)floor((double)J.n_red * l_rate);
    L.identity = 0;
    if (n_ls == 0) {
      n_ls = J.n_red;
      L.identity = 1;
    }
    J.n_ls = n_ls;
    L.seed = J.seed;
    L.domain = PSULVSB_DOMAIN_L_SAMPLED;
    L.event = (uint32_t)J.host_round;
    L.n = J.n_red;
    L.count = n_ls;
    L.max_draws = L.identity ? 0ull : sample_max_draws_formula(L.n, L.count);
    L.first = J.first;
    L.chunk_prefix = J.chunk_prefix;
    L.ticket = J.ticket;
    L.draws = J.draws;
    L.draws_cap = J.draws_cap;
    L.blist = J.blist;
    L.blist_cap = J.blist_cap;
    L.bcount = J.bcount;
    L.out = J.L_sampled;
    L.status = &J.sample_status[0];
    L.post = 1;
    L.vbits = J.vbits;
    L.edges = J.edges;
    L.via = nullptr;
    L.gathered = nullptr;
    L.flags = J.sampled_flags;
    L.n_points = J.C;
    L.active = 1;
    J.sample_status[0] = 1ull;
    J.phase = PHASE_LOCAL;
    prepare_local(J, sb[blockIdx.x], gj[blockIdx.x], cq[blockIdx.x], P);
  }
}

__global__ void __launch_bounds__(BLK)
    engine_scale_kernel(JobCtl* __restrict__ jobs, GncJob* __restrict__ gj, CliqueJob* __restrict__ cq, EngineParams P) {
  JobCtl& J = jobs[blockIdx.x];
  if (J.phase != PHASE_LOCAL || !J.estimate_scaling) return;
  __shared__ BlockScratch scratch;
  __shared__ double est_s, scale_s;
  __shared__ int base_s;
  const int tid = threadIdx.x;
  const int K = J.basic_choose;
  const uint2* __restrict__ edges = J.basic_edges;
  double* __restrict__ X = J.weights;
  double* __restrict__ A = J.lv;
  const double beta = 2.0 * J.cur.noise_bound * sqrt(J.cur.cbar2);
  double scale = J.cur_scale;
  int n_pruned = 0;
  if (K > 0) {
    for (int i = tid; i < K; i += BLK) {
      const uint2 e = edges[i];
      const double* sa = J.src + 3 * (size_t)e.x;
      const double* sb = J.src + 3 * (size_t)e.y;
      const double* ta = J.dst + 3 * (size_t)e.x;
      const double* tb = J.dst + 3 * (size_t)e.y;
      const double v1 = sqrt(sqnorm3(dsub(sb[0], sa[0]), dsub(sb[1], sa[1]), dsub(sb[2], sa[2])));
      const double v2 = sqrt(sqnorm3(dsub(tb[0], ta[0]), dsub(tb[1], ta[1]), dsub(tb[2], ta[2])));
      X[i] = v2 / v1;
      A[i] = dmul(beta, 1.0 / v1);
    }
    block_tls_scale(&scratch, X, A, K, J.seed, (uint32_t)J.scale_calls, !J.first_time, J.last_best.s, scale, &est_s,
                    &scale_s);
    const double est = est_s;
    scale = scale_s;
    if (tid == 0) base_s = 0;
    __syncthreads();
    for (int i0 = 0; i0 < K; i0 += BLK) {
      const int i = i0 + tid;
      const int f = (i < K && fabs(dsub(X[i], est)) <= A[i]) ? 1 : 0;
      int ea, eb, ta, tb;
      block_scan2(&scratch, f, 0, ea, eb, ta, tb);
      const int base = base_s;
      if (f) J.pruned_edges[base + ea] = edges[i];
      __syncthreads();
      if (tid == 0) base_s = base + ta;
      __syncthreads();
    }
    n_pruned = base_s;
  }
  __syncthreads();
  if (tid == 0) {
    if (K > 0) J.scale_calls += 1;
    J.scale_noise = beta;
    J.cur_scale = scale;
    J.n_pruned = n_pruned;
    GncJob& g = gj[blockIdx.x];
    g.edges = J.pruned_edges;
    g.K = (unsigned long long)n_pruned;
    g.inv_scale = 1.0 / scale;
    g.noise_bound = J.cur.noise_bound * (2.0 / scale);
    CliqueJob& q = cq[blockIdx.x];
    q.edges = J.pruned_edges;
    q.n_edges = (unsigned long long)n_pruned;
    q.filter = 0;
  }
}

__device__ __forceinline__ void host_score_point(JobCtl& J, const EngineParams& P, const Xform& X, const uint32_t ev,
                                                 const int j, int& add, int& imap, int& inl) {
    const double res = residual_ref(J.ori_src + 3 * (size_t)j, J.ori_dst + 3 * (size_t)j, X.s, X.R, X.t);
    if (res <= J.tau) {
      inl = 1;
      J.inlier_counter[j] += 1;
      const int km = J.keep_mask[j];
      if (km == 0) {
        const int hst = J.inlier_history[j];
        if (hst == -1 || hst == 1)
          add = 1;
        else if (hst == 0)
          add = (philox_uniform01(J.seed, PSULVSB_DOMAIN_UNIFORM, ev, (uint64_t)j) <=
                 inlier_probability(res, P.score_sigma))
                    ? 1
                    : 0;
      }
      if (add) {
        J.final_inliers[j] = 1;
      } else if (km == 1) {
        imap = 1;
        J.final_inliers[j] = 1;
      }
      J.inlier_history[j] = 1;
    } else {
      const double u = philox_uniform01(J.seed, PSULVSB_DOMAIN_UNIFORM, ev, (uint64_t)j);
      if (u > inlier_probability(J.residual_history[j], P.score_sigma)) J.final_inliers[j] = 0;
      J.inlier_history[j] = 0;
    }
    J.residual_history[j] = res;
}

__device__ void finish_host_round(JobCtl& J, const EngineParams& P, const Xform& X, const int curr, const double elapsed_s,
                                  SampleJob& sbj, GncJob& gjj, CliqueJob& cqj, int* __restrict__ n_done,
                                  const int new_corr_count, const int inlier_map_size) {
  const int M = J.M;
  J.host_r += J.local_r;
  J.host_scorings += 1;
  J.new_corr_count = new_corr_count;
  J.inlier_map_size = inlier_map_size;
  const double b_now = kBRate[J.rate_idx];
  if (curr > J.best_host_cnt || J.pro_host == 0.0 || (b_now == 1.0 && curr >= J.best_host_cnt)) {
    J.best_host = X;
    J.best_host_cnt = curr;
  }
  J.last_best = J.best_host;
  J.pro_host = 1.0 - pow(1.0 - (double)((double)J.best_host_cnt / (double)M), J.host_r);
  const bool timeup = P.wallclock_cap_s > 0.0 && elapsed_s > P.wallclock_cap_s;
  if (J.pro_host > P.tpro_host || J.longholi || timeup) J.pro_host_not_over = 0;
  if (kLRate[J.rate_idx] == 1.0 && b_now == 1.0) J.longholi = 1;
  if (J.host_trace && J.n_host_trace < J.host_trace_cap) {
    psulvsb_host_trace_t& T = J.host_trace[J.n_host_trace++];
    T.host_round = J.host_round;
    T.curr_count = curr;
    T.best_host = J.best_host_cnt;
    T.new_corr_count = P.self_update ? J.new_corr_count : 0;
    T.inlier_map_size = J.inlier_map_size;
    T.host_r = J.host_r;
    T.p_host = J.pro_host;
  }
  J.host_round += 1;
  sbj.active = 0;
  gjj.active = 0;
  cqj.active = 0;
  if (J.pro_host_not_over && J.rounds_left > 0) {
    J.phase = PHASE_ROUND_START;
    atomicAdd(n_done + 1, 1);
  } else {
    J.valid = 1;
    J.phase = PHASE_DONE;
    atomicAdd(n_done, 1);
  }
}

__global__ void __launch_bounds__(BLK)
    engine_local_control_kernel(JobCtl* __restrict__ jobs, SampleJob* __restrict__ sl, SampleJob* __restrict__ sb,
                                GncJob* __restrict__ gj, CliqueJob* __restrict__ cq, EngineParams P, double elapsed_s,
                                int* __restrict__ n_done) {
  JobCtl& J = jobs[blockIdx.x];
  if (J.phase != PHASE_LOCAL) return;
  __shared__ BlockScratch scratch;
  __shared__ int base_s[2];
  __shared__ int similar_s;
  __shared__ Xform sol_s;
  const int tid = threadIdx.x;
  const int C = J.C;
  const double b_rate = kBRate[J.rate_idx];
  const bool clique_round = (b_rate == 1.0);

// ... 433 lines not shown
```

probabilistic-self-update-line-vector-set-based-point-cloud-registration_b200/csrc/engine_kernels.cuh:

```cuda
#pragma once

#include "engine.cuh"
#include "engine_state.cuh"

namespace psulvsb {

constexpr int kCtlThreads = 1024;

__global__ void engine_init_kernel(JobCtl* jobs, SampleJob* sl, SampleJob* sb, GncJob* gj, CliqueJob* cq,
                                   const unsigned long long* n_edges, EngineParams P, int* n_done);
__global__ void engine_round_start_kernel(JobCtl* jobs, SampleJob* sl, SampleJob* sb, GncJob* gj, CliqueJob* cq,
                                          EngineParams P, int* n_done);
__global__ void engine_scale_kernel(JobCtl* jobs, GncJob* gj, CliqueJob* cq, EngineParams P);
__global__ void engine_local_control_kernel(JobCtl* jobs, SampleJob* sl, SampleJob* sb, GncJob* gj, CliqueJob* cq,
                                            EngineParams P, double elapsed_s, int* n_done);
__global__ void engine_host_score_kernel(JobCtl* jobs, EngineParams P);
__global__ void engine_host_finish_kernel(JobCtl* jobs, SampleJob* sb, GncJob* gj, CliqueJob* cq, EngineParams P,
                                          double elapsed_s, int* n_done);
__global__ void engine_refine_kernel(JobCtl* jobs, psulvsb_solution_t* out, const unsigned long long* border);
__global__ void engine_export_points_kernel(const JobCtl* jobs, int job, int* final_inliers, int* inlier_counter);

}
```

probabilistic-self-update-line-vector-set-based-point-cloud-registration_b200/csrc/engine_state.cuh:

```cuda
#pragma once

#include <cuda_runtime.h>
#include <stdint.h>

#include "engine.cuh"

namespace psulvsb {

enum : int { PHASE_ROUND_START = 0, PHASE_LOCAL = 1, PHASE_DONE = 2,
             PHASE_HOST_SCORE = 3 };

struct Xform {
  double s;
  double R[9];
  double t[3];
};

struct SubParams {
  double noise_bound, cbar2;
  int max_iterations;
  double gnc_factor, cost_threshold;
};

struct EngineParams {
  SubParams caller, inloop;
  int sampler_counters;
  int zero_sampler_scratch;
  double pr_noise;
  double score_sigma;
  double rotation_similar;
  int local_max_iter;
  double tpro_host, tpro_local;
  int host_round_limit;
  double wallclock_cap_s;
  int self_update;
  int inlier_selection_mode;
  int max_local_iters;
  int split_host_scoring;
};

struct JobCtl {
  int C0, M, Ccap;
  double* src;
  double* dst;
  const double* src0;
  const double* dst0;
  const double* ori_src;
  const double* ori_dst;
  const int* keep_mask0;
  const int* reduce_map0;
  int* keep_mask;
  int* reduce_map;
  int* inlier_counter;
  int* new_corr;
  int* inlier_history;
  int* final_inliers;
  uint32_t* hs_bits;
  int hs_curr;
  double* residual_history;
  int* inlier_map;
  int* idx;
  double* xs;
  double* xs_sorted;
  uint8_t* sampled_flags;
  uint8_t* rot_flags;
  uint2* edges;
  unsigned long long edge_cap;
  uint32_t* vbits;
  uint32_t* blist;
  unsigned long long blist_cap;
  unsigned int* bcount;
  uint32_t* first;
  unsigned long long first_words;
  uint32_t* draws;
  unsigned long long draws_cap;
  unsigned long long* chunk_prefix;
  unsigned int* ticket;
  uint32_t* L_sampled;
  uint32_t* basic_idx;
  uint2* basic_edges;
  double* weights;
  double* lv;
  unsigned long long lv_cap;
  double* pts8;
  uint32_t* gnc_perm;
  double* gnc_grid_red;
  unsigned int* gnc_grid_bar;
  uint32_t* adj;
  int adj_stride;
  uint8_t* clique_flags;
  uint2* pruned_edges;
  int estimate_scaling;
  psulvsb_local_trace_t* local_trace;
  psulvsb_host_trace_t* host_trace;
  int local_trace_cap, host_trace_cap;
  uint64_t seed;
  double tau;
  int C;
  unsigned long long n_red, n_red0, n_ls;
  int n_sampled_pts, basic_choose;
  int phase, status;
  int rounds_left, host_round, local_iter_global, host_scorings, escalations;
  int first_time, sampled_first_time, inloop, longholi, rate_idx;
  int local_r, host_r, best_sampled_cnt, best_host_cnt;
  double pro_local, pro_host;
  int pro_host_not_over;
  double scale_noise, translation_noise;
  Xform sol, best_sampled, best_host, last_best;
  int new_corr_count, inlier_map_size;
  int scale_calls, n_pruned;
  int clique_size, clique_proven, aborted;
  double cur_scale;
  unsigned long long sample_status[2];
  double R_gnc[9];
  int gnc_info[4];
  double gnc_cost;
  SubParams cur;
  int n_local_trace, n_host_trace;
  int valid, refined;
};

}
```

probabilistic-self-update-line-vector-set-based-point-cloud-registration_b200/csrc/k1_consistency.cu:

```cuda
#include <cuda_runtime.h>

#include <type_traits>

#include <cstdlib>

#include "common.cuh"
#include "engine.cuh"

namespace psulvsb {

namespace {

constexpr int K1_THREADS = 256;
#ifndef K1_COLPAIR_UNROLL
#define K1_COLPAIR_UNROLL 4
#endif
#ifndef K1_R4_CTAS
#define K1_R4_CTAS 2
#endif

__device__ __forceinline__ bool exact_consistent(const double* __restrict__ s64, const double* __restrict__ t64, int i,
                                                 int j, double beta) {
  const double sx = dsub(s64[3 * j + 0], s64[3 * i + 0]);
  const double sy = dsub(s64[3 * j + 1], s64[3 * i + 1]);
// ... 279 lines not shown
      else if (R > 2 && n_live == 2)
        eval_word<(R > 2 ? 2 : 1), R>(cw, tw, ms, mt, two_beta2, beta4, acc, mv);
      else
        eval_word<(R > 3 ? 3 : 1), R>(cw, tw, ms, mt, two_beta2, beta4, acc, mv);
      auto finish = [&](auto full_tag) {
        constexpr bool FULL = decltype(full_tag)::value;
        const uint32_t valid = (FULL || cb + 32 <= n) ? 0xFFFFFFFFu : ((1u << (n - cb)) - 1u);
        uint32_t live[R], word[R];
        bool doubt = false;
#pragma unroll
        for (int r = 0; r < R; ++r) {
          const int i = irow[r];
          const uint32_t upper =
              (FULL || i < cb) ? 0xFFFFFFFFu : ((i >= cb + 31) ? 0u : (0xFFFFFFFFu << (i - cb + 1)));
          live[r] = FULL ? row_ok[r] : (row_ok[r] & valid & upper);
          word[r] = acc[r] & live[r];
          doubt = doubt || (live[r] != 0u && !(mv[r] > t_fast));
        }
        if (__ballot_sync(0xffffffffu, doubt) != 0u) {
#pragma unroll
          for (int r = 0; r < R; ++r) {
            unsigned int flagged = __ballot_sync(0xffffffffu, live[r] != 0u && !(mv[r] > t_fast));
            while (flagged) {
              const int owner = __ffs(flagged) - 1;
              flagged &= flagged - 1;
              const int oi = __shfl_sync(0xffffffffu, irow[r], owner);
              const float4 si = make_float4(-0.5f * __shfl_sync(0xffffffffu, ms[r].x, owner),
                                            -0.5f * __shfl_sync(0xffffffffu, ms[r].y, owner),
                                            -0.5f * __shfl_sync(0xffffffffu, ms[r].z, owner), 0.f);
              const float4 ti = make_float4(-0.5f * __shfl_sync(0xffffffffu, mt[r].x, owner),
                                            -0.5f * __shfl_sync(0xffffffffu, mt[r].y, owner),
                                            -0.5f * __shfl_sync(0xffffffffu, mt[r].z, owner), 0.f);
              const uint32_t res =
                  slow_word_coop(slow, oi, cb, si, ti, il_load(&cs[st][wj * 32], lane), il_load(&ct[st][wj * 32], lane), nborder);
              if (lane == owner) word[r] = res & live[r];
            }
          }
        }
#pragma unroll
        for (int r = 0; r < R; ++r) {
          if (row_sectors) {
            sw[(wj * R + r) * 32] = word[r];
          } else if (row_ok[r]) {
            mask[(size_t)irow[r] * stride + (cb >> 5)] = word[r];
          }
          cnt[r] += __popc(word[r]);
        }
      };
      if (cb >= row0 + TI && cb + 32 <= n)
        finish(std::true_type());
      else
        finish(std::false_type());
    }
    if (row_sectors) {
#pragma unroll
      for (int r = 0; r < R; ++r)
        if (irow[r] < row_end) {
          uint4 lo, hi;
          lo.x = sw[(0 * R + r) * 32];
          lo.y = sw[(1 * R + r) * 32];
          lo.z = sw[(2 * R + r) * 32];
          lo.w = sw[(3 * R + r) * 32];
          hi.x = sw[(4 * R + r) * 32];
          hi.y = sw[(5 * R + r) * 32];
          hi.z = sw[(6 * R + r) * 32];
          hi.w = sw[(7 * R + r) * 32];
          uint4* __restrict__ out = reinterpret_cast<uint4*>(mask + (size_t)irow[r] * stride + (col0 >> 5));
          out[0] = lo;
          out[1] = hi;
        }
    }
    __syncwarp();
    if (lane == 0) mbar_arrive(&bar_empty[st]);
  }
#pragma unroll
  for (int r = 0; r < R; ++r)
    if (irow[r] < row_end && cnt[r] != 0u && row_counts) atomicAdd(&row_counts[irow[r]], cnt[r]);
  if (border_count) {
    unsigned int tot = (unsigned int)warp_sum_int((int)nborder);
    if ((tid & 31) == 0 && tot) atomicAdd(border_count, (unsigned long long)tot);
  }
}

__global__ void pack_points_kernel(const double* __restrict__ pts, int n, double cx, double cy, double cz,
                                   float4* __restrict__ out) {
  const int i = blockIdx.x * blockDim.x + threadIdx.x;
  if (i < n) out[i] = pack_point(pts[3 * i] - cx, pts[3 * i + 1] - cy, pts[3 * i + 2] - cz);
}

__global__ void interleave_points_kernel(const float4* __restrict__ in, int n, float4* __restrict__ out) {
  const int i = blockIdx.x * blockDim.x + threadIdx.x;
  if (i < n) il_store(out, i, in[i]);
  if (i == n && (n & 1)) il_store(out, n, make_float4(0.f, 0.f, 0.f, 0.f));
}

__global__ void symmetrize_kernel(uint32_t* __restrict__ mask, int n, int stride, int nblk) {
  const int warp = (blockIdx.x * blockDim.x + threadIdx.x) >> 5;
  const int lane = threadIdx.x & 31;
  const long long total = (long long)nblk * (nblk + 1) / 2;
  if (warp >= total) return;
  int bi = (int)((sqrt(8.0 * (double)warp + 1.0) - 1.0) * 0.5);
  while ((long long)bi * (bi + 1) / 2 > warp) --bi;
  while ((long long)(bi + 1) * (bi + 2) / 2 <= warp) ++bi;
  const int bj = warp - (int)((long long)bi * (bi + 1) / 2);
  const int jrow = bj * 32 + lane;
  const uint32_t s = (jrow < n) ? mask[(size_t)jrow * stride + bi] : 0u;
  uint32_t mine = 0u;
#pragma unroll
  for (int b = 0; b < 32; ++b) {
    const uint32_t t = __ballot_sync(0xffffffffu, (s >> b) & 1u);
    if (lane == b) mine = t;
  }
  const int irow = bi * 32 + lane;
  if (irow < n) {
    uint32_t* dstw = &mask[(size_t)irow * stride + bj];
    if (bi == bj)
      *dstw = *dstw | mine;
    else
      *dstw = mine;
  }
}

__global__ void __launch_bounds__(1024) row_scan_kernel(const CompactJob* __restrict__ jobs) {
  const CompactJob& job = jobs[blockIdx.x];
  if (!job.active) return;
  const uint32_t* __restrict__ counts = job.row_counts;
  unsigned long long* __restrict__ offsets = job.offsets;
  const int n = job.n;
  __shared__ unsigned long long part[1024];
  const int tid = threadIdx.x;
  const int per = (n + 1023) / 1024;
  const int lo = min(n, tid * per), hi = min(n, lo + per);
  unsigned long long s = 0;
  for (int i = lo; i < hi; ++i) s += counts[i];
  part[tid] = s;
  __syncthreads();
  for (int off = 1; off < 1024; off <<= 1) {
    unsigned long long v = (tid >= off) ? part[tid - off] : 0ull;
    __syncthreads();
    part[tid] += v;
    __syncthreads();
  }
  unsigned long long run = part[tid] - s;
  for (int i = lo; i < hi; ++i) {
    offsets[i] = run;
    run += counts[i];
  }
  if (tid == 1023) {
    offsets[n] = part[1023];
    if (job.n_edges) *job.n_edges = part[1023];
  }
}

__global__ void compact_edges_kernel(const CompactJob* __restrict__ jobs) {
  const CompactJob& job = jobs[blockIdx.y];
  if (!job.active || !job.edges) return;
  const uint32_t* __restrict__ mask = job.mask;
  const int n = job.n, stride = job.stride;
  const unsigned long long cap = job.cap;
  uint2* __restrict__ edges = job.edges;
  const int row = (int)(((long long)blockIdx.x * blockDim.x + threadIdx.x) >> 5);
  const int lane = threadIdx.x & 31;
  if (row >= n) return;
  if (job.row_counts && job.row_counts[row] == 0u) return;
  const int W = (n + 31) >> 5;
  unsigned long long base = job.offsets[row];
  for (int w0 = row >> 5; w0 < W; w0 += 32) {
    const int w = w0 + lane;
    uint32_t word = (w < W) ? mask[(size_t)row * stride + w] : 0u;
    const int pc = __popc(word);
    int incl = pc;
#pragma unroll
    for (int o = 1; o < 32; o <<= 1) {
      int t = __shfl_up_sync(0xffffffffu, incl, o);
      if (lane >= o) incl += t;
    }
    unsigned long long pos = base + (unsigned long long)(incl - pc);
    while (word) {
      const int b = __ffs(word) - 1;
      word &= word - 1;
      if (pos < cap) edges[pos] = make_uint2((unsigned)row, (unsigned)(w * 32 + b));
      ++pos;
    }
    base += (unsigned long long)__shfl_sync(0xffffffffu, incl, 31);
  }
}

}

K1Consts make_k1_consts(double beta, double coord_bound) {
  const double mu = 5.9604644775390625e-08;
  const double cmax = coord_bound > beta ? coord_bound : beta;
  const double b2 = beta * beta;
  double cpad = b2 / 64.0;
  const double need = 32.0 * mu * (b2 + beta * cmax);
  if (need > cpad) cpad = need;
  const double cc = b2 + cpad;
  K1Consts k;
  k.half_bias = (float)(0.5 * cc);
  k.two_beta2 = (float)(2.0 * b2);
  k.r0 = (float)(2.0 * b2 * cc - b2 * b2);
  const double kappa = 384.0 * mu * beta * cmax;
  k.kappa = (float)(kappa * 1.0001);
  k.w_thr = (float)(kappa * cc * 1.01 + 1e-30);
  k.beta = beta;
  const double C2 = cmax * cmax;
  const double E = 80.0 * mu * C2;
  const double ED = 2.0 * E + 12.0 * mu * C2;
  const double ES = 2.0 * E + 24.0 * mu * C2;
  const double c0 = ED * ED + 2.0 * b2 * ES + 2.0 * mu * (48.0 * b2 * C2 + b2 * b2);
  const double Dlim = ED + sqrt(ED * ED + 48.0 * b2 * C2 + c0) + b2;
  const double Terr = 2.0 * Dlim * ED + c0;
  k.beta4 = (float)(b2 * b2);
  k.t_fast = (float)((Terr + 2.0 * b2 * b2) * 1.05 + 1e-30);
  return k;
}

template <int R, int TJ, bool SECT>
static int launch_k1_variant(cudaStream_t st, const K1Job* d_jobs, int n_jobs, int max_n, int max_rows) {
  constexpr int TI = K1_THREADS * R;
  const int n_tiles = (max_n + TJ - 1) / TJ;
  const int row_blocks = (max_rows + TI - 1) / TI;
  const double live_tiles = 0.55 * (double)n_tiles * row_blocks * n_jobs;
  int tpc = (int)(live_tiles / ((double)sm_count() * 3.0 * 12.0));
  if (tpc < 1) tpc = 1;
  if (tpc > 16) tpc = 16;
  if (R == 4 && tpc >= 3) tpc = (tpc + 3) / 4 * 4;
  if (tpc > n_tiles) tpc = n_tiles;
  dim3 grid((n_tiles + tpc - 1) / tpc, row_blocks, n_jobs);
  constexpr int stage_bytes = (K1_THREADS / 32) * (TJ / 32) * R * 32 * (int)sizeof(uint32_t);
  static bool attr_set = false;
  if (!attr_set) {
    PSU_CUDA(cudaFuncSetAttribute(k1_mask_kernel<R, TJ, SECT>, cudaFuncAttributeMaxDynamicSharedMemorySize, stage_bytes));
    attr_set = true;
  }
  k1_mask_kernel<R, TJ, SECT><<<grid, K1_THREADS, stage_bytes, st>>>(d_jobs, tpc);
  PSU_CHECK_LAUNCH("k1_mask_kernel");
  return PSULVSB_OK;
}

int launch_consistency_mask(cudaStream_t st, const K1Job* d_jobs, int n_jobs, int max_n, int max_rows, bool row_sectors) {
  if (n_jobs <= 0 || max_n < 1 || max_rows < 1) return PSULVSB_OK;
  const double pairs = 0.5 * (double)max_rows * max_n * n_jobs;
  int variant = pairs >= 5.0e8 ? 4 : (pairs >= 1.0e8 ? 2 : 1);
  if (debug_knobs().k1_variant >= 1 && debug_knobs().k1_variant <= 4) variant = debug_knobs().k1_variant;
  if (row_sectors) {
    if (variant == 3) return launch_k1_variant<3, 256, true>(st, d_jobs, n_jobs, max_n, max_rows);
    if (variant == 4) return launch_k1_variant<4, 256, true>(st, d_jobs, n_jobs, max_n, max_rows);
    if (variant == 2) return launch_k1_variant<2, 256, true>(st, d_jobs, n_jobs, max_n, max_rows);
    return launch_k1_variant<1, 256, true>(st, d_jobs, n_jobs, max_n, max_rows);
  }
  if (variant == 3) return launch_k1_variant<3, 256, false>(st, d_jobs, n_jobs, max_n, max_rows);
  if (variant == 4) return launch_k1_variant<4, 256, false>(st, d_jobs, n_jobs, max_n, max_rows);
  if (variant == 2) return launch_k1_variant<2, 256, false>(st, d_jobs, n_jobs, max_n, max_rows);
  return launch_k1_variant<1, 256, false>(st, d_jobs, n_jobs, max_n, max_rows);
}

int launch_pack_points(cudaStream_t st, const double* pts, int n, const double center[3], float4* out) {
  if (n <= 0) return PSULVSB_OK;
  const double cx = center ? center[0] : 0.0, cy = center ? center[1] : 0.0, cz = center ? center[2] : 0.0;
  pack_points_kernel<<<(n + 255) / 256, 256, 0, st>>>(pts, n, cx, cy, cz, out);
  PSU_CHECK_LAUNCH("pack_points_kernel");
  return PSULVSB_OK;
}

int launch_interleave_points(cudaStream_t st, const float4* in, int n, float4* out) {
  if (n <= 0) return PSULVSB_OK;
  interleave_points_kernel<<<(n + 1 + 255) / 256, 256, 0, st>>>(in, n, out);
  PSU_CHECK_LAUNCH("interleave_points_kernel");
  return PSULVSB_OK;
}

int launch_symmetrize(cudaStream_t st, uint32_t* mask, int n, int stride) {
  const int nblk = (n + 31) / 32;
  const long long warps = (long long)nblk * (nblk + 1) / 2;
  const long long threads = warps * 32;
  symmetrize_kernel<<<(unsigned)((threads + 255) / 256), 256, 0, st>>>(mask, n, stride, nblk);
  PSU_CHECK_LAUNCH("symmetrize_kernel");
  return PSULVSB_OK;
}

int launch_compact_edges(cudaStream_t st, const CompactJob* d_jobs, int n_jobs, int max_n, bool scan, bool emit) {
  if (n_jobs <= 0 || max_n < 1) return PSULVSB_OK;
  if (scan) {
    row_scan_kernel<<<n_jobs, 1024, 0, st>>>(d_jobs);
    PSU_CHECK_LAUNCH("row_scan_kernel");
  }
  if (emit) {
    const long long threads = (long long)max_n * 32;
    dim3 grid((unsigned)((threads + 255) / 256), n_jobs);
    compact_edges_kernel<<<grid, 256, 0, st>>>(d_jobs);
    PSU_CHECK_LAUNCH("compact_edges_kernel");
  }
  return PSULVSB_OK;
}

}
```

probabilistic-self-update-line-vector-set-based-point-cloud-registration_b200/csrc/k1_ratio.cu:

```cuda
#include <cuda_runtime.h>

#include <climits>
#include <functional>
#include <string>
#include <vector>

#include "common.cuh"
#include "engine.cuh"

namespace psulvsb {

namespace {

constexpr int RB_THREADS = 256;
constexpr int RB_SMEM_BINS = 2048;
constexpr double kMaxScale0 = 10000.0;
constexpr double kBinSize = 20.0;

__device__ __forceinline__ unsigned long long row_offset(unsigned long long i, unsigned long long n) {
  return i * (2ull * n - i - 1ull) / 2ull;
}

__device__ __forceinline__ double pair_ratio(const double* __restrict__ s, const double* __restrict__ t, int i, int j) {
  const double sx = dsub(s[3 * j + 0], s[3 * i + 0]), sy = dsub(s[3 * j + 1], s[3 * i + 1]),
// ... 125 lines not shown
    const uint32_t b = ratio_bin(X, grown ? scale_at(job, l) : kMaxScale0);
    job.pair_bin[l] = b;
    if (b < RB_SMEM_BINS)
      atomicAdd(&sh[b], 1u);
    else
      atomicAdd(&job.hist[b], 1u);
  }
  __syncthreads();
  for (int k = threadIdx.x; k < RB_SMEM_BINS; k += RB_THREADS)
    if (sh[k]) atomicAdd(&job.hist[k], sh[k]);
}

__global__ void __launch_bounds__(1024) ratio_max_kernel(const RatioJob* __restrict__ jobs) {
  const RatioJob& job = jobs[blockIdx.x];
  if (!job.active) return;
  __shared__ unsigned int wmax[32];
  unsigned int m = 0;
  const long long hsize = (long long)(*job.final_scale * kBinSize);
  for (long long b = threadIdx.x; b < hsize; b += 1024) m = max(m, job.hist[b]);
#pragma unroll
  for (int o = 16; o > 0; o >>= 1) m = max(m, __shfl_xor_sync(0xffffffffu, m, o));
  if ((threadIdx.x & 31) == 0) wmax[threadIdx.x >> 5] = m;
  __syncthreads();
  if (threadIdx.x == 0) {
    unsigned int mm = 0;
    for (int w = 0; w < 32; ++w) mm = max(mm, wmax[w]);
    job.peak[0] = mm;
    job.peak[1] = 0xFFFFFFFFu;
  }
}

__global__ void __launch_bounds__(RB_THREADS) ratio_last_kernel(const RatioJob* __restrict__ jobs) {
  const RatioJob& job = jobs[blockIdx.y];
  if (!job.active) return;
  const unsigned long long L = (unsigned long long)job.n * (unsigned long long)(job.n - 1) / 2ull;
  const unsigned int mh = job.peak[0];
  for (unsigned long long l = (unsigned long long)blockIdx.x * RB_THREADS + threadIdx.x; l < L;
       l += (unsigned long long)gridDim.x * RB_THREADS) {
    const uint32_t b = job.pair_bin[l];
    if (job.hist[b] == mh) atomicMax(&job.last[b], l + 1ull);
  }
}

__global__ void __launch_bounds__(1024) ratio_peak_kernel(const RatioJob* __restrict__ jobs) {
  const RatioJob& job = jobs[blockIdx.x];
  if (!job.active) return;
  __shared__ unsigned long long wbest[32];
  __shared__ unsigned int wbin[32];
  const unsigned int mh = job.peak[0];
  unsigned long long best = ~0ull;
  unsigned int bin = 0xFFFFFFFFu;
  const long long hsize = (long long)(*job.final_scale * kBinSize);
  for (long long b = threadIdx.x; b < hsize; b += 1024)
    if (job.hist[b] == mh && mh > 0) {
      const unsigned long long last = job.last[b];
      if (last < best) {
        best = last;
        bin = (unsigned int)b;
      }
    }
#pragma unroll
  for (int o = 16; o > 0; o >>= 1) {
    const unsigned long long ob = __shfl_xor_sync(0xffffffffu, best, o);
    const unsigned int obin = __shfl_xor_sync(0xffffffffu, bin, o);
    if (ob < best) {
      best = ob;
      bin = obin;
    }
  }
  if ((threadIdx.x & 31) == 0) {
    wbest[threadIdx.x >> 5] = best;
    wbin[threadIdx.x >> 5] = bin;
  }
  __syncthreads();
  if (threadIdx.x == 0) {
    for (int w = 0; w < 32; ++w)
      if (wbest[w] < best) {
        best = wbest[w];
        bin = wbin[w];
      }
    job.peak[1] = bin;
  }
}

__device__ __forceinline__ int bin_class(uint32_t b, uint32_t peak, uint32_t hsize) {
  if (b == peak) return 0;
  if (peak != 0u && b == peak - 1u) return 1;
  if (peak != hsize - 1u && b == peak + 1u) return 2;
  return 3;
}

__global__ void __launch_bounds__(256) ratio_class_count_kernel(const RatioJob* __restrict__ jobs) {
  const RatioJob& job = jobs[blockIdx.y];
  if (!job.active) return;
  const int n = job.n;
  const int row = (int)(((long long)blockIdx.x * blockDim.x + threadIdx.x) >> 5);
  const int lane = threadIdx.x & 31;
  if (row >= n) return;
  const uint32_t peak = job.peak[1];
  const uint32_t hsize = (uint32_t)(*job.final_scale * kBinSize);
  unsigned int c0 = 0, c1 = 0, c2 = 0;
  if (row < n - 1 && peak != 0xFFFFFFFFu) {
    const unsigned long long base = row_offset((unsigned long long)row, (unsigned long long)n);
    const int len = n - 1 - row;
    for (int k = lane; k < len; k += 32) {
      const int c = bin_class(job.pair_bin[base + k], peak, hsize);
      c0 += c == 0;
      c1 += c == 1;
      c2 += c == 2;
    }
  }
#pragma unroll
  for (int o = 16; o > 0; o >>= 1) {
    c0 += __shfl_xor_sync(0xffffffffu, c0, o);
    c1 += __shfl_xor_sync(0xffffffffu, c1, o);
    c2 += __shfl_xor_sync(0xffffffffu, c2, o);
  }
  if (lane == 0) {
    job.class_counts[row] = c0;
    job.class_counts[n + row] = c1;
    job.class_counts[2 * n + row] = c2;
  }
}

__global__ void __launch_bounds__(1024) ratio_class_scan_kernel(const RatioJob* __restrict__ jobs) {
  const RatioJob& job = jobs[blockIdx.x];
  if (!job.active) return;
  const int m = 3 * job.n;
  __shared__ unsigned long long part[1024];
  const int tid = threadIdx.x;
  const int per = (m + 1023) / 1024;
  const int lo = min(m, tid * per), hi = min(m, lo + per);
  unsigned long long s = 0;
  for (int i = lo; i < hi; ++i) s += job.class_counts[i];
  part[tid] = s;
  __syncthreads();
  for (int off = 1; off < 1024; off <<= 1) {
    const unsigned long long v = (tid >= off) ? part[tid - off] : 0ull;
    __syncthreads();
    part[tid] += v;
    __syncthreads();
  }
  unsigned long long run = part[tid] - s;
  for (int i = lo; i < hi; ++i) {
    job.class_offsets[i] = run;
    run += job.class_counts[i];
  }
  if (tid == 1023) {
    job.class_offsets[m] = part[1023];
    *job.n_edges = part[1023];
  }
}

__global__ void __launch_bounds__(256) ratio_class_emit_kernel(const RatioJob* __restrict__ jobs) {
  const RatioJob& job = jobs[blockIdx.y];
  if (!job.active || !job.edges) return;
  const int n = job.n;
  const int row = (int)(((long long)blockIdx.x * blockDim.x + threadIdx.x) >> 5);
  const int lane = threadIdx.x & 31;
  if (row >= n - 1) return;
  const uint32_t peak = job.peak[1];
  if (peak == 0xFFFFFFFFu) return;
  const uint32_t hsize = (uint32_t)(*job.final_scale * kBinSize);
  const unsigned long long base = row_offset((unsigned long long)row, (unsigned long long)n);
  const int len = n - 1 - row;
  unsigned long long pos[3] = {job.class_offsets[row], job.class_offsets[n + row], job.class_offsets[2 * n + row]};
  for (int k0 = 0; k0 < len; k0 += 32) {
    const int k = k0 + lane;
    const int c = (k < len) ? bin_class(job.pair_bin[base + k], peak, hsize) : 3;
#pragma unroll
    for (int cc = 0; cc < 3; ++cc) {
      const unsigned int m = __ballot_sync(0xffffffffu, c == cc);
      if (c == cc) {
        const unsigned long long p = pos[cc] + (unsigned long long)__popc(m & ((1u << lane) - 1u));
        if (p < job.cap) job.edges[p] = make_uint2((unsigned)row, (unsigned)(row + 1 + k));
      }
      pos[cc] += (unsigned long long)__popc(m);
    }
  }
}

}

static int launch_ratio_reduced_set(cudaStream_t st, const RatioJob* d_jobs, int n_jobs, int max_n, int phase) {
  if (n_jobs <= 0 || max_n < 2) return PSULVSB_OK;
  const long long row_threads = (long long)max_n * 32;
  const dim3 row_grid((unsigned)((row_threads + 255) / 256), (unsigned)n_jobs);
  if (phase == 0) {
    ratio_rowmax_kernel<<<dim3((unsigned)(max_n - 1), (unsigned)n_jobs), RB_THREADS, 0, st>>>(d_jobs);
    PSU_CHECK_LAUNCH("ratio_rowmax_kernel");
    ratio_growth_kernel<<<n_jobs, RG_THREADS, 0, st>>>(d_jobs);
    PSU_CHECK_LAUNCH("ratio_growth_kernel");
  } else if (phase == 1) {
    ratio_bins_kernel<<<dim3((unsigned)(max_n - 1), (unsigned)n_jobs), RB_THREADS, 0, st>>>(d_jobs);
    PSU_CHECK_LAUNCH("ratio_bins_kernel");
    ratio_max_kernel<<<n_jobs, 1024, 0, st>>>(d_jobs);
    PSU_CHECK_LAUNCH("ratio_max_kernel");
    const unsigned long long L = (unsigned long long)max_n * (unsigned long long)(max_n - 1) / 2ull;
    unsigned long long gx = (L + RB_THREADS * 8 - 1) / (RB_THREADS * 8);
    if (gx > sm_count() * 16) gx = sm_count() * 16;
    if (gx < 1) gx = 1;
    ratio_last_kernel<<<dim3((unsigned)gx, (unsigned)n_jobs), RB_THREADS, 0, st>>>(d_jobs);
    PSU_CHECK_LAUNCH("ratio_last_kernel");
    ratio_peak_kernel<<<n_jobs, 1024, 0, st>>>(d_jobs);
    PSU_CHECK_LAUNCH("ratio_peak_kernel");
    ratio_class_count_kernel<<<row_grid, 256, 0, st>>>(d_jobs);
    PSU_CHECK_LAUNCH("ratio_class_count_kernel");
    ratio_class_scan_kernel<<<n_jobs, 1024, 0, st>>>(d_jobs);
    PSU_CHECK_LAUNCH("ratio_class_scan_kernel");
  } else {
    ratio_class_emit_kernel<<<row_grid, 256, 0, st>>>(d_jobs);
    PSU_CHECK_LAUNCH("ratio_class_emit_kernel");
  }
  return PSULVSB_OK;
}

int ratio_count(cudaStream_t st, std::vector<RatioJob>& rj, RatioJob* d_rj, int max_n,
                const std::function<void*(size_t)>& hist_arena, cudaEvent_t ev0, cudaEvent_t ev1) {
  const int B = (int)rj.size();
  PSU_CUDA(cudaMemcpyAsync(d_rj, rj.data(), sizeof(RatioJob) * (size_t)B, cudaMemcpyHostToDevice, st));
  if (int rc = launch_ratio_reduced_set(st, d_rj, B, max_n, 0)) return rc;
  std::vector<double> fscale((size_t)B);
  std::vector<int> bad((size_t)B);
  PSU_CUDA(cudaMemcpyAsync(fscale.data(), rj[0].final_scale, sizeof(double) * (size_t)B, cudaMemcpyDeviceToHost, st));
  PSU_CUDA(cudaMemcpyAsync(bad.data(), rj[0].bad, sizeof(int) * (size_t)B, cudaMemcpyDeviceToHost, st));
  PSU_CUDA(cudaStreamSynchronize(st));
  size_t bins_total = 0;
  for (int b = 0; b < B; ++b) {
    if (bad[(size_t)b])
      return fail(PSULVSB_ERR_UNSUPPORTED,
                  "problem " + std::to_string(b) +
                      (bad[(size_t)b] == 1 ? ": an infinite length ratio (coincident source points with distinct targets; "
                                             "registration.cc:714-718 is undefined there)"
                                           : ": the ratio histogram would outgrow the supported MaxScale of 2e6 "
                                             "(registration.cc:714-718)"));
    bins_total += (size_t)(fscale[(size_t)b] * kBinSize) + 64;
  }
  const size_t bytes = bins_total * (sizeof(unsigned int) + sizeof(unsigned long long));
  char* hb = static_cast<char*>(hist_arena(bytes));
  if (!hb) return PSULVSB_ERR_CUDA;
  size_t off = 0;
  for (int b = 0; b < B; ++b) {
    rj[(size_t)b].last = reinterpret_cast<unsigned long long*>(hb + off);
    off += ((size_t)(fscale[(size_t)b] * kBinSize) + 64) * sizeof(unsigned long long);
  }
  for (int b = 0; b < B; ++b) {
    rj[(size_t)b].hist = reinterpret_cast<unsigned int*>(hb + off);
    off += ((size_t)(fscale[(size_t)b] * kBinSize) + 64) * sizeof(unsigned int);
  }
  PSU_CUDA(cudaMemsetAsync(hb, 0, off, st));
  PSU_CUDA(cudaMemcpyAsync(d_rj, rj.data(), sizeof(RatioJob) * (size_t)B, cudaMemcpyHostToDevice, st));
  if (ev0) PSU_CUDA(cudaEventRecord(ev0, st));
  if (int rc = launch_ratio_reduced_set(st, d_rj, B, max_n, 1)) return rc;
  if (ev1) PSU_CUDA(cudaEventRecord(ev1, st));
  return PSULVSB_OK;
}

int ratio_emit(cudaStream_t st, const std::vector<RatioJob>& rj, RatioJob* d_rj, int max_n) {
  PSU_CUDA(cudaMemcpyAsync(d_rj, rj.data(), sizeof(RatioJob) * rj.size(), cudaMemcpyHostToDevice, st));
  return launch_ratio_reduced_set(st, d_rj, (int)rj.size(), max_n, 2);
}

}
```

probabilistic-self-update-line-vector-set-based-point-cloud-registration_b200/csrc/k2_sampler.cu:

```cuda
#include <cstdlib>
#include <cuda_runtime.h>

#include "common.cuh"
#include "engine.cuh"

namespace psulvsb {

namespace {

constexpr int SMP_THREADS = 256;
constexpr int SMP_CHUNK = SMP_THREADS * 4;
constexpr int SMB_THREADS = 1024;
constexpr int SMP_BW = 49152;
constexpr int SMP_MAX_LIST_BUCKETS = 512;

struct ListPlan {
  unsigned int n_buckets, w_bits, width;
  unsigned int wide;
  unsigned long long cap_b;
};
__host__ __device__ inline unsigned long long list_cap_for(unsigned long long n, unsigned long long max_draws,
                                                          unsigned long long width) {
  const unsigned long long mean = (max_draws * width + n - 1) / n + 1;
  unsigned long long s = 1;
  while (s * s < mean) ++s;
  return (mean + 10 * s + 64 + 3) & ~3ull;
}
__host__ __device__ inline bool sample_list_plan(unsigned long long n, unsigned long long max_draws,
                                                 unsigned long long blist_cap, ListPlan& p) {
  p.n_buckets = 0;
  p.cap_b = 0;
  p.wide = 0;
  if (max_draws < 2 || n < 3ull * SMP_BW) return false;
  unsigned int k_bits = 1;
  while (((max_draws - 1) >> k_bits) != 0ull) ++k_bits;
  if (k_bits <= 24) {
    p.w_bits = 32u - k_bits;
    p.width = (p.w_bits >= 16u) ? (unsigned int)SMP_BW : (1u << p.w_bits);
    const unsigned long long nb = (n + p.width - 1) / p.width;
    if (nb >= 3 && nb <= (unsigned long long)SMP_MAX_LIST_BUCKETS) {
      p.n_buckets = (unsigned int)nb;
      p.cap_b = list_cap_for(n, max_draws, p.width);
      if (nb * p.cap_b <= blist_cap) return true;
    }
  }
  if (k_bits > 32) return false;
  p.w_bits = 32u;
  p.width = (unsigned int)SMP_BW;
  const unsigned long long nbw = (n + SMP_BW - 1) / SMP_BW;
  if (nbw < 3 || nbw > (unsigned long long)SMP_MAX_LIST_BUCKETS) {
    p.n_buckets = 0;
    p.cap_b = 0;
    return false;
  }
  p.n_buckets = (unsigned int)nbw;
  p.cap_b = list_cap_for(n, max_draws, p.width);
  p.wide = 1;
  return 2ull * nbw * p.cap_b <= blist_cap;
}
__device__ __forceinline__ uint32_t list_bucket(uint32_t v, const ListPlan& p) {
  return (p.w_bits >= 16u) ? v / (uint32_t)SMP_BW : v >> p.w_bits;
}

struct FastMod {
  unsigned long long magic;
  uint32_t n;
};
__device__ __forceinline__ FastMod make_fastmod(uint32_t n) {
  FastMod f;
  f.n = n;
  f.magic = n > 1u ? (~0ull / n) + 1ull : 0ull;
  return f;
}
__device__ __forceinline__ uint32_t draw_value(uint32_t word, const FastMod& f) {
  const uint32_t v = word >> 1;
  if (f.n <= 1u) return 0u;
  const uint32_t q = (uint32_t)__umul64hi((unsigned long long)v, f.magic);
  return v - q * f.n;
}

__global__ void __launch_bounds__(256) sample_draws_kernel(const SampleJob* __restrict__ jobs, unsigned int list_cap_test) {
  const SampleJob& job = jobs[blockIdx.y];
  if (!job.active || job.identity) return;
  const bool cache = job.draws != nullptr && job.max_draws <= job.draws_cap;
  const unsigned long long nblocks = (job.max_draws + 3) >> 2;
  if ((unsigned long long)blockIdx.x * 256 >= nblocks) return;
  __shared__ ListPlan plan_s;
  __shared__ FastMod fm_s;
  __shared__ int lists_s;
  if (threadIdx.x == 0) {
    lists_s = (job.blist != nullptr && sample_list_plan(job.n, job.max_draws, job.blist_cap, plan_s)) ? 1 : 0;
    fm_s = make_fastmod((uint32_t)job.n);
  }
  __syncthreads();
  const ListPlan plan = plan_s;
  const bool lists = lists_s != 0;
  const unsigned int n_buckets = plan.n_buckets;
  const unsigned long long cap_b = plan.cap_b;
  const unsigned long long cap_fill = (list_cap_test != 0u && list_cap_test < plan.cap_b) ? list_cap_test : plan.cap_b;
  if (!cache && !lists) return;
  const FastMod fm = fm_s;
  uint4* __restrict__ out = reinterpret_cast<uint4*>(job.draws);
  if (!lists) {
    for (unsigned long long q = (unsigned long long)blockIdx.x * 256 + threadIdx.x; q < nblocks;
         q += (unsigned long long)gridDim.x * 256) {
      const Philox4 o = philox4x32_10(job.seed, job.domain, job.event, q);
      out[q] = make_uint4(draw_value(o.w[0], fm), draw_value(o.w[1], fm), draw_value(o.w[2], fm), draw_value(o.w[3], fm));
    }
    return;
  }
  constexpr int QPT = 4;
  __shared__ unsigned int wh[8][SMP_MAX_LIST_BUCKETS];
  __shared__ unsigned int base[SMP_MAX_LIST_BUCKETS];
  const int tid = threadIdx.x, lane = tid & 31, wid = tid >> 5;
  const unsigned int lt_mask = (1u << lane) - 1u;
  const unsigned long long max_draws = job.max_draws;
  for (unsigned long long q0 = (unsigned long long)blockIdx.x * (256 * QPT); q0 < nblocks;
       q0 += (unsigned long long)gridDim.x * (256 * QPT)) {
    uint32_t vv[QPT][4];
    unsigned int rk[QPT][4];
    for (int b = lane; b < (int)n_buckets; b += 32) wh[wid][b] = 0u;
#pragma unroll
    for (int u = 0; u < QPT; ++u) {
      const unsigned long long q = q0 + (unsigned long long)u * 256 + tid;
#pragma unroll
      for (int l = 0; l < 4; ++l) vv[u][l] = 0xFFFFFFFFu;
      if (q < nblocks) {
        const Philox4 o = philox4x32_10(job.seed, job.domain, job.event, q);
        uint32_t v4[4];
#pragma unroll
        for (int l = 0; l < 4; ++l) v4[l] = draw_value(o.w[l], fm);
        if (cache) out[q] = make_uint4(v4[0], v4[1], v4[2], v4[3]);
#pragma unroll
        for (int l = 0; l < 4; ++l)
          if ((q << 2) + l < max_draws) vv[u][l] = v4[l];
      }
    }
    __syncwarp();
#pragma unroll
    for (int u = 0; u < QPT; ++u)
#pragma unroll
      for (int l = 0; l < 4; ++l) {
        const uint32_t b = (vv[u][l] != 0xFFFFFFFFu) ? list_bucket(vv[u][l], plan) : 0xFFFFFFFFu;
        const unsigned int peers = __match_any_sync(0xffffffffu, b);
        const int leader = __ffs(peers) - 1;
        unsigned int start = 0u;
        if (lane == leader && b != 0xFFFFFFFFu) {
          start = wh[wid][b];
          wh[wid][b] = start + __popc(peers);
        }
        start = __shfl_sync(0xffffffffu, start, leader);
        rk[u][l] = start + __popc(peers & lt_mask);
        __syncwarp();
      }
    __syncthreads();
    for (int bk = tid; bk < (int)n_buckets; bk += 256) {
      unsigned int run = 0u;
#pragma unroll
      for (int w = 0; w < 8; ++w) {
        const unsigned int c = wh[w][bk];
        wh[w][bk] = run;
        run += c;
      }
      if (run != 0u) base[bk] = atomicAdd(&job.bcount[bk], run);
    }
    __syncthreads();
#pragma unroll
// ... 100 lines not shown
      const unsigned int bn = b + gridDim.x;
      if (bn < n_buckets) fetch(bn, nxt, cnt_nxt);
      const uint32_t* __restrict__ list = job.blist + (unsigned long long)b * plan.cap_b;
      if (vbits)
        for (uint32_t i = tid; i < (plan.width >> 5); i += SMB_THREADS) wbm[i] = 0u;
      __syncthreads();
#pragma unroll
      for (int j = 0; j < EPT; ++j)
        if (tid + j * SMB_THREADS < cnt_cur) atomicMin(&table[cur[j] & wmask], cur[j] >> wb);
      for (uint32_t i = tid + EPT * SMB_THREADS; i < cnt_cur; i += SMB_THREADS) {
        const uint32_t e = __ldcg(list + i);
        atomicMin(&table[e & wmask], e >> wb);
      }
      __syncthreads();
      const uint32_t lo_b = b * plan.width;
#pragma unroll
      for (int j = 0; j < EPT; ++j)
        if (tid + j * SMB_THREADS < cnt_cur) {
          const uint32_t k = cur[j] >> wb;
          if (table[cur[j] & wmask] == k) {
            atomicOr(&accept[k >> 5], 1u << (k & 31));
            if (vbits) atomicOr(&wbm[(cur[j] & wmask) >> 5], 1u << (cur[j] & 31u));
          }
        }
      for (uint32_t i = tid + EPT * SMB_THREADS; i < cnt_cur; i += SMB_THREADS) {
        const uint32_t e = __ldcg(list + i);
        const uint32_t k = e >> wb;
        if (table[e & wmask] == k) {
          atomicOr(&accept[k >> 5], 1u << (k & 31));
          if (vbits) atomicOr(&wbm[(e & wmask) >> 5], 1u << (e & 31u));
        }
      }
      __syncthreads();
      if (vbits)
        for (uint32_t i = tid; i < (plan.width >> 5); i += SMB_THREADS)
          if (wbm[i] && ((unsigned long long)lo_b + 32ull * i) < job.n) vbits[(lo_b >> 5) + i] = wbm[i];
#pragma unroll
      for (int j = 0; j < EPT; ++j)
        if (tid + j * SMB_THREADS < cnt_cur) table[cur[j] & wmask] = 0xFFFFFFFFu;
      for (uint32_t i = tid + EPT * SMB_THREADS; i < cnt_cur; i += SMB_THREADS) table[__ldcg(list + i) & wmask] = 0xFFFFFFFFu;
      if (tid == 0) job.bcount[b] = 0u;
#pragma unroll
      for (int j = 0; j < EPT; ++j) cur[j] = nxt[j];
      cnt_cur = cnt_nxt;
    }
  } else {
  if (list_mode && blockIdx.x == 0)
    for (int i = tid; i < SMP_MAX_LIST_BUCKETS; i += SMB_THREADS) job.bcount[i] = 0u;
  for (unsigned int b = blockIdx.x; b < n_buckets; b += gridDim.x) {
    const uint32_t lo = b * (uint32_t)SMP_BW;
    const uint32_t width = min((uint32_t)SMP_BW, n - lo);
    __syncthreads();
    for (uint32_t i = tid; i < width; i += SMB_THREADS) table[i] = 0xFFFFFFFFu;
    if (vbits)
      for (uint32_t i = tid; i < (uint32_t)(SMP_BW / 32); i += SMB_THREADS) wbm[i] = 0u;
    __syncthreads();
    const uint32_t nb32 = (uint32_t)nblocks, md32 = (uint32_t)max_draws;
    for (uint32_t q0 = tid; q0 < nb32; q0 += 4 * SMB_THREADS) {
      uint4 d4[4];
#pragma unroll
      for (int u = 0; u < 4; ++u) {
        const uint32_t q = q0 + u * SMB_THREADS;
        d4[u] = q < nb32 ? draws_of(q) : make_uint4(0xFFFFFFFFu, 0xFFFFFFFFu, 0xFFFFFFFFu, 0xFFFFFFFFu);
      }
#pragma unroll
      for (int u = 0; u < 4; ++u) {
        const uint32_t q = q0 + u * SMB_THREADS;
        const uint32_t vv[4] = {d4[u].x, d4[u].y, d4[u].z, d4[u].w};
#pragma unroll
        for (int l = 0; l < 4; ++l) {
          const uint32_t k = (q << 2) + l;
          const uint32_t off = vv[l] - lo;
          if (off < width && k < md32) atomicMin(&table[off], k);
        }
      }
    }
    __syncthreads();
    for (uint32_t q0 = tid; q0 < nb32; q0 += 4 * SMB_THREADS) {
      uint4 d4[4];
#pragma unroll
      for (int u = 0; u < 4; ++u) {
        const uint32_t q = q0 + u * SMB_THREADS;
        d4[u] = q < nb32 ? draws_of(q) : make_uint4(0xFFFFFFFFu, 0xFFFFFFFFu, 0xFFFFFFFFu, 0xFFFFFFFFu);
      }
#pragma unroll
      for (int u = 0; u < 4; ++u) {
        const uint32_t q = q0 + u * SMB_THREADS;
        const uint32_t vv[4] = {d4[u].x, d4[u].y, d4[u].z, d4[u].w};
        uint32_t bits = 0u;
#pragma unroll
        for (int l = 0; l < 4; ++l) {
          const uint32_t k = (q << 2) + l;
          const uint32_t off = vv[l] - lo;
          if (off < width && k < md32 && table[off] == k) {
            bits |= 1u << l;
            if (vbits) atomicOr(&wbm[off >> 5], 1u << (off & 31u));
          }
        }
        if (bits) atomicOr(&accept[q >> 3], bits << ((q & 7) << 2));
      }
    }
    if (vbits) {
      __syncthreads();
      for (uint32_t i = tid; i < ((width + 31u) >> 5); i += SMB_THREADS)
        if (wbm[i]) vbits[(lo >> 5) + i] = wbm[i];
    }
  }
  }
  __threadfence();
  __syncthreads();
  if (tid == 0) ticket_s = atomicAdd(job.ticket, 1u);
  __syncthreads();
  if (ticket_s != n_workers - 1) return;
  __threadfence();
  if (tid == 0) {
    carry_s = 0ull;
    *job.ticket = 0u;
    if (job.blist != nullptr) job.bcount[SMP_MAX_LIST_BUCKETS] = 0u;
  }
  __syncthreads();
  const unsigned long long nchunks = (max_draws + SMP_CHUNK - 1) / SMP_CHUNK;
  constexpr int WPC = SMP_CHUNK / 32;
  const unsigned long long nwords = (max_draws + 31) >> 5;
  for (unsigned long long c0 = 0; c0 < nchunks; c0 += SMB_THREADS) {
    const unsigned long long ch = c0 + tid;
    unsigned int v = 0;
    if (ch < nchunks)
      for (int w = 0; w < WPC; ++w) {
        const unsigned long long wi = ch * WPC + w;
        if (wi < nwords) v += __popc(__ldcg(accept + wi));
      }
    const int lane = tid & 31, wid = tid >> 5;
    unsigned int incl = v;
#pragma unroll
    for (int o = 1; o < 32; o <<= 1) {
      const unsigned int t = __shfl_up_sync(0xffffffffu, incl, o);
      if (lane >= o) incl += t;
    }
    if (lane == 31) sh[wid] = incl;
    __syncthreads();
    unsigned int wbase = 0;
#pragma unroll
    for (int w = 0; w < SMB_THREADS / 32; ++w)
      if (w < wid) wbase += sh[w];
    const unsigned long long carry = carry_s;
    if (ch < nchunks) job.chunk_prefix[ch] = carry + wbase + (incl - v);
    __syncthreads();
    if (tid == SMB_THREADS - 1) carry_s = carry + wbase + incl;
    __syncthreads();
  }
  if (tid == 0 && carry_s < job.count && job.status) job.status[0] = 0ull;
}

__global__ void __launch_bounds__(SMP_THREADS) sample_emit_kernel(const SampleJob* __restrict__ jobs) {
  const SampleJob& job = jobs[blockIdx.y];
  if (!job.active) return;
  __shared__ unsigned int sh[SMP_THREADS / 32];
  const int tid = threadIdx.x, lane = tid & 31, wid = tid >> 5;
  const unsigned long long count = job.count;
  uint32_t* __restrict__ out = job.out;
  if (job.identity) {
    for (unsigned long long r = (unsigned long long)blockIdx.x * SMP_THREADS + tid; r < count;
         r += (unsigned long long)gridDim.x * SMP_THREADS) {
      out[r] = (uint32_t)r;
      if (job.post == 1) {
        const uint2 e = job.edges[r];
        job.flags[e.x] = 1;
        job.flags[e.y] = 1;
      } else if (job.post == 2) {
        job.gathered[r] = job.edges[job.via[r]];
      }
    }
    if (blockIdx.x == 0 && tid == 0 && job.status) job.status[0] = 1ull;
    return;
  }
  const FastMod fm = make_fastmod((uint32_t)job.n);
  const unsigned long long max_draws = job.max_draws;
  const unsigned long long nchunks = (max_draws + SMP_CHUNK - 1) / SMP_CHUNK;
  const unsigned long long nwords = (max_draws + 31) >> 5;
  const bool cached = job.draws != nullptr && max_draws <= job.draws_cap;
  uint32_t* __restrict__ accept = job.first;
  for (unsigned long long ch = blockIdx.x; ch < nchunks; ch += gridDim.x) {
    const unsigned long long q = ch * SMP_THREADS + tid;
    const unsigned long long wi = q >> 3;
    const uint32_t word = (wi < nwords) ? __ldcg(accept + wi) : 0u;
    const uint32_t bits = (word >> ((q & 7) << 2)) & 0xFu;
    const unsigned int c = __popc(bits);
    unsigned int incl = c;
#pragma unroll
    for (int o = 1; o < 32; o <<= 1) {
      const unsigned int t = __shfl_up_sync(0xffffffffu, incl, o);
      if (lane >= o) incl += t;
    }
    if (lane == 31) sh[wid] = incl;
    __syncthreads();
    unsigned int wbase = 0;
#pragma unroll
    for (int w = 0; w < SMP_THREADS / 32; ++w)
      if (w < wid) wbase += sh[w];
    if ((q & 7) == 0 && wi < nwords && word != 0u) accept[wi] = 0u;
    unsigned long long rank = job.chunk_prefix[ch] + wbase + (incl - c);
    if (bits) {
      uint32_t vv[4];
      if (cached) {
        const uint4 d4 = __ldcg(reinterpret_cast<const uint4*>(job.draws) + q);
        vv[0] = d4.x; vv[1] = d4.y; vv[2] = d4.z; vv[3] = d4.w;
      } else {
        const Philox4 o = philox4x32_10(job.seed, job.domain, job.event, q);
#pragma unroll
        for (int l = 0; l < 4; ++l) vv[l] = draw_value(o.w[l], fm);
      }
#pragma unroll
      for (int l = 0; l < 4; ++l) {
        if ((bits >> l) & 1u) {
          if (rank < count) {
            const uint32_t v = vv[l];
            out[rank] = v;
            if (job.post == 1 && !job.vbits) {
              const uint2 e = job.edges[v];
              job.flags[e.x] = 1;
              job.flags[e.y] = 1;
            } else if (job.post == 2) {
              const uint2 e = job.edges[job.via[v]];
              job.gathered[rank] = e;
              if (job.lv_out && rank < job.lv_cap) {
                const double2* pa = reinterpret_cast<const double2*>(job.pts8 + 8 * (size_t)e.x);
                const double2* pb = reinterpret_cast<const double2*>(job.pts8 + 8 * (size_t)e.y);
                const double2 a0 = __ldg(pa), a1 = __ldg(pa + 1), a2 = __ldg(pa + 2);
                const double2 b0 = __ldg(pb), b1 = __ldg(pb + 1), b2 = __ldg(pb + 2);
                double* __restrict__ o = job.lv_out + rank;
                const size_t st = (size_t)job.lv_cap;
                __stcg(o, b0.x - a0.x);
                __stcg(o + st, b0.y - a0.y);
                __stcg(o + 2 * st, b1.x - a1.x);
                __stcg(o + 3 * st, b1.y - a1.y);
                __stcg(o + 4 * st, b2.x - a2.x);
                __stcg(o + 5 * st, b2.y - a2.y);
              }
            }
            if (rank == count - 1 && job.status) job.status[0] = (q << 2) + l + 1;
          } else if (job.post == 1 && job.vbits) {
            atomicAnd(&job.vbits[vv[l] >> 5], ~(1u << (vv[l] & 31u)));
          }
          ++rank;
        }
      }
    }
    __syncthreads();
  }
}

__global__ void __launch_bounds__(256) sample_flag_kernel(const SampleJob* __restrict__ jobs) {
  const SampleJob& job = jobs[blockIdx.y];
  if (!job.active || job.identity || job.post != 1 || !job.vbits) return;
  const unsigned long long nwords = (job.n + 31) >> 5;
  const unsigned long long threads = (unsigned long long)gridDim.x * 256;
  const uint2* __restrict__ edges = job.edges;
  for (unsigned long long wi = (unsigned long long)blockIdx.x * 256 + threadIdx.x; wi < nwords; wi += threads) {
    uint32_t word = __ldcg(job.vbits + wi);
    if (!word) continue;
    job.vbits[wi] = 0u;
    const uint2* __restrict__ row = edges + wi * 32;
    while (word) {
      uint2 e[4];
      int m = 0;
#pragma unroll
      for (int j = 0; j < 4; ++j) {
        if (word) {
          const int bit = __ffs(word) - 1;
          word &= word - 1;
          e[j] = row[bit];
          m = j + 1;
        }
      }
#pragma unroll
      for (int j = 0; j < 4; ++j)
        if (j < m) {
          job.flags[e[j].x] = 1;
          job.flags[e[j].y] = 1;
        }
    }
  }
}

__global__ void philox_fill_kernel(uint64_t seed, uint32_t domain, uint32_t event, unsigned long long first_k,
                                   unsigned long long count, uint32_t* __restrict__ out) {
  const unsigned long long i = (unsigned long long)blockIdx.x * blockDim.x + threadIdx.x;
  if (i < count) out[i] = philox_rand31(seed, domain, event, first_k + i);
}

}

unsigned long long sample_default_max_draws(unsigned long long n, unsigned long long count) {
  return sample_max_draws_formula(n, count);
}

unsigned long long sample_list_entries(unsigned long long n, unsigned long long max_draws) {
  ListPlan p;
  if (!sample_list_plan(n, max_draws, ~0ull, p)) return 0;
  return (unsigned long long)p.n_buckets * p.cap_b * (p.wide ? 2ull : 1ull);
}
unsigned long long sample_list_counters() { return SMP_MAX_LIST_BUCKETS + 4; }

unsigned long long sample_chunk_slots(unsigned long long max_draws) { return (max_draws + SMP_CHUNK - 1) / SMP_CHUNK + 1; }

unsigned long long sample_table_words(unsigned long long n, unsigned long long max_draws) {
  (void)n;
  return (max_draws + 31) / 32 + 8;
}

int launch_sample(cudaStream_t st, const SampleJob* d_jobs, int n_jobs, unsigned long long max_draws_bound,
                  unsigned long long n_bound, bool flag_pass) {
  if (n_jobs <= 0) return PSULVSB_OK;
  static bool attr_set = false;
  const size_t smem = (size_t)SMP_BW * 4 + (size_t)SMP_BW / 8;
  if (!attr_set) {
    PSU_CUDA(cudaFuncSetAttribute(sample_bucket_kernel, cudaFuncAttributeMaxDynamicSharedMemorySize, (int)smem));
    attr_set = true;
  }
  const unsigned long long nchunks = (max_draws_bound + SMP_CHUNK - 1) / SMP_CHUNK;
  unsigned long long gx = nchunks;
  const unsigned long long cap = (unsigned long long)(sm_count() * 16) / (unsigned long long)(n_jobs < 64 ? n_jobs : 64) + 1;
  if (gx > cap) gx = cap;
  if (gx < 1) gx = 1;
  const unsigned int list_cap_test = (unsigned int)debug_knobs().sample_list_cap_test;
  sample_draws_kernel<<<dim3((unsigned)gx, (unsigned)n_jobs), 256, 0, st>>>(d_jobs, list_cap_test);
  PSU_CHECK_LAUNCH("sample_draws_kernel");
  unsigned long long nb = (n_bound + SMP_BW - 1) / SMP_BW;
  if (nb < 1) nb = 1;
  unsigned long long bx = ((unsigned long long)sm_count() * 3ull + (unsigned long long)n_jobs - 1) / (unsigned long long)n_jobs;
  if (bx > nb) bx = nb;
  if (bx < 1) bx = 1;
  sample_bucket_kernel<<<dim3((unsigned)bx, (unsigned)n_jobs), SMB_THREADS, smem, st>>>(d_jobs);
  PSU_CHECK_LAUNCH("sample_bucket_kernel");
  sample_emit_kernel<<<dim3((unsigned)gx, (unsigned)n_jobs), SMP_THREADS, 0, st>>>(d_jobs);
  PSU_CHECK_LAUNCH("sample_emit_kernel");
  if (flag_pass) {
    unsigned long long fx = (n_bound + 32ull * 256 - 1) / (32ull * 256);
    const unsigned long long fcap = ((unsigned long long)sm_count() * 16 + (unsigned long long)n_jobs - 1) / (unsigned long long)n_jobs;
    if (fx > fcap) fx = fcap;
    if (fx < 1) fx = 1;
    sample_flag_kernel<<<dim3((unsigned)fx, (unsigned)n_jobs), 256, 0, st>>>(d_jobs);
    PSU_CHECK_LAUNCH("sample_flag_kernel");
  }
  return PSULVSB_OK;
}

int launch_philox_fill(cudaStream_t st, uint64_t seed, uint32_t domain, uint32_t event, unsigned long long first_k,
                       unsigned long long count, uint32_t* out) {
  if (count == 0) return PSULVSB_OK;
  philox_fill_kernel<<<(unsigned)((count + 255) / 256), 256, 0, st>>>(seed, domain, event, first_k, count, out);
  PSU_CHECK_LAUNCH("philox_fill_kernel");
  return PSULVSB_OK;
}

}
```

Baseline: 15520.

## Pack edges into 32-bit pairs and flag sampled points via shared-memory bitmap

Adds a narrow 16+16-bit edge format used when all correspondence counts fit in 16 bits, templating the compaction, ratio emit, round-start, sample emit and flag kernels on the edge format. This halves the edge buffer traffic. The flag kernel now collects touched points in a shared-memory bitmap and writes the byte flags in bulk, and the compaction kernel prefetches the next mask word. It adds template instantiations and a per-CTA bitmap zero and flush, which may cost more than it saves for small point counts.

```diff
diff --git a/probabilistic-self-update-line-vector-set-based-point-cloud-registration_b200/csrc/capi.cu b/probabilistic-self-update-line-vector-set-based-point-cloud-registration_b200/csrc/capi.cu
--- a/probabilistic-self-update-line-vector-set-based-point-cloud-registration_b200/csrc/capi.cu
+++ b/probabilistic-self-update-line-vector-set-based-point-cloud-registration_b200/csrc/capi.cu
@@ -194,6 +194,7 @@
   else if (n == "sample_list_cap_test") k.sample_list_cap_test = (int)value;
   else if (n == "k1_variant") k.k1_variant = (int)value;
   else if (n == "upload_prof") k.upload_prof = (int)value;
+  else if (n == "edge_wide") k.edge_wide = (int)value;
   else if (n == "reset") k = DebugKnobs();
   else return fail(PSULVSB_ERR_INVALID, "psulvsb_debug_set: unknown switch " + n);
   return PSULVSB_OK;
@@ -305,13 +306,13 @@
   j.stride = row_stride_words;
   j.row_counts = d_row_counts;
   j.offsets = d_row_offsets;
-  j.edges = (uint2*)d_edges_uint2;
+  j.edges = d_edges_uint2;
   j.cap = edge_capacity;
   j.n_edges = d_n_edges;
   j.active = 1;
   DeviceJob<CompactJob> dj(st);
   if (int rc = dj.put(j)) return rc;
-  return launch_compact_edges(st, dj.d, 1, n, true, d_edges_uint2 != nullptr);
+  return launch_compact_edges(st, dj.d, 1, n, true, d_edges_uint2 != nullptr, false);
 }
 
 int psulvsb_ratio_reduced_set(void* stream, const double* d_src64, const double* d_dst64, int n, uint32_t* d_pair_bin,
@@ -390,9 +391,9 @@
   if (ne > edge_capacity)
     return fail(PSULVSB_ERR_CAPACITY, "psulvsb_ratio_reduced_set: " + std::to_string(ne) + " edges, capacity " +
                                           std::to_string(edge_capacity));
-  j.edges = (uint2*)d_edges_uint2;
+  j.edges = d_edges_uint2;
   j.cap = edge_capacity;
-  if (int rc = ratio_emit(st, rj, dj.d, n)) return rc;
+  if (int rc = ratio_emit(st, rj, dj.d, n, false)) return rc;
   PSU_CUDA(cudaStreamSynchronize(st));
   return PSULVSB_OK;
 }
diff --git a/probabilistic-self-update-line-vector-set-based-point-cloud-registration_b200/csrc/common.cuh b/probabilistic-self-update-line-vector-set-based-point-cloud-registration_b200/csrc/common.cuh
--- a/probabilistic-self-update-line-vector-set-based-point-cloud-registration_b200/csrc/common.cuh
+++ b/probabilistic-self-update-line-vector-set-based-point-cloud-registration_b200/csrc/common.cuh
@@ -43,6 +43,7 @@
   int sample_list_cap_test = 0;
   int k1_variant = 0;
   int upload_prof = 0;
+  int edge_wide = 0;
 };
 DebugKnobs& debug_knobs();
 
diff --git a/probabilistic-self-update-line-vector-set-based-point-cloud-registration_b200/csrc/edge_fmt.cuh b/probabilistic-self-update-line-vector-set-based-point-cloud-registration_b200/csrc/edge_fmt.cuh
--- /dev/null
+++ b/probabilistic-self-update-line-vector-set-based-point-cloud-registration_b200/csrc/edge_fmt.cuh
@@ -0,0 +1,34 @@
+#pragma once
+#include <cstddef>
+#include <cstdint>
+#include <cuda_runtime.h>
+
+namespace psulvsb {
+
+struct EdgeWide {
+  using T = uint2;
+  __device__ __forceinline__ static uint2 load(const void* p, unsigned long long k) {
+    return static_cast<const uint2*>(p)[k];
+  }
+  __device__ __forceinline__ static void store(void* p, unsigned long long k, unsigned int i, unsigned int j) {
+    static_cast<uint2*>(p)[k] = make_uint2(i, j);
+  }
+};
+
+struct EdgeNarrow {
+  using T = uint32_t;
+  __device__ __forceinline__ static uint2 load(const void* p, unsigned long long k) {
+    const uint32_t e = static_cast<const uint32_t*>(p)[k];
+    return make_uint2(e >> 16, e & 0xFFFFu);
+  }
+  __device__ __forceinline__ static void store(void* p, unsigned long long k, unsigned int i, unsigned int j) {
+    static_cast<uint32_t*>(p)[k] = (i << 16) | j;
+  }
+};
+
+constexpr long long kEdgeNarrowMaxPoints = 65536;
+
+inline bool edge_narrow_fits(long long ccap) { return ccap <= kEdgeNarrowMaxPoints; }
+inline size_t edge_bytes(bool narrow) { return narrow ? sizeof(EdgeNarrow::T) : sizeof(EdgeWide::T); }
+
+}
diff --git a/probabilistic-self-update-line-vector-set-based-point-cloud-registration_b200/csrc/engine.cu b/probabilistic-self-update-line-vector-set-based-point-cloud-registration_b200/csrc/engine.cu
--- a/probabilistic-self-update-line-vector-set-based-point-cloud-registration_b200/csrc/engine.cu
+++ b/probabilistic-self-update-line-vector-set-based-point-cloud-registration_b200/csrc/engine.cu
@@ -669,7 +669,7 @@
       if (int rc = launch_consistency_mask(st, m.k1, B, maxC, sharded ? row_e - row_b : maxC, true)) return rc;
     PSU_CUDA(cudaEventRecord(ev_m1, st));
     ++launches;
-    if (int rc = launch_compact_edges(st, m.cj, B, maxC, true, false)) return rc;
+    if (int rc = launch_compact_edges(st, m.cj, B, maxC, true, false, false)) return rc;
     ++launches;
   }
   if (int rc = h_small.ensure((sizeof(unsigned long long) + sizeof(int)) * (size_t)B + 64 + 66 * sizeof(unsigned long long)))
@@ -693,6 +693,8 @@
     PSU_CUDA(cudaStreamSynchronize(st));
   }
 
+  bool narrow = !sharded && !debug_knobs().edge_wide;
+  for (int b = 0; b < B; ++b) narrow = narrow && edge_narrow_fits(lay[(size_t)(b0 + b)].Ccap);
   const int grid_ctas_max = sm_count() / (B > 0 ? B : 1);
   unsigned long long max_cap = 0, max_nred = 0;
   {
@@ -704,7 +706,7 @@
         unsigned long long cap = h_nedges[b] + reserve[(size_t)(b0 + b)];
         if (cap < 64) cap = 64;
         J.edge_cap = cap;
-        J.edges = be.take<uint2>((size_t)cap);
+        J.edges = narrow ? (void*)be.take<EdgeNarrow::T>((size_t)cap) : (void*)be.take<EdgeWide::T>((size_t)cap);
         J.first_words = sample_table_words(cap, sample_default_max_draws(cap, cap));
         J.first = be.take<uint32_t>((size_t)J.first_words);
         J.draws_cap = (cap + 3) & ~3ull;
@@ -731,7 +733,7 @@
           rj[(size_t)b].edges = J.edges;
           rj[(size_t)b].cap = cap;
         }
-        cj[(size_t)b].edges = J.edges + (sharded && be.base ? shard_off[(size_t)comm_rank(comm)] : 0ull);
+        cj[(size_t)b].edges = static_cast<EdgeWide::T*>(J.edges) + (sharded && be.base ? shard_off[(size_t)comm_rank(comm)] : 0ull);
         cj[(size_t)b].cap = cap - (sharded ? shard_off[(size_t)comm_rank(comm)] : 0ull);
         max_cap = cap > max_cap ? cap : max_cap;
         max_nred = h_nedges[b] > max_nred ? h_nedges[b] : max_nred;
@@ -745,10 +747,10 @@
   if (max_cap >= 0x7FFFFFF0ull) return fail(PSULVSB_ERR_UNSUPPORTED, "reduced set exceeds the 31-bit sample / line-vector indices");
   PSU_CUDA(cudaMemcpyAsync(m.jobs, jobs.data(), sizeof(JobCtl) * (size_t)B, cudaMemcpyHostToDevice, st));
   if (ratio) {
-    if (int rc = ratio_emit(st, rj, m.rj, maxC)) return rc;
+    if (int rc = ratio_emit(st, rj, m.rj, maxC, narrow)) return rc;
   } else {
     PSU_CUDA(cudaMemcpyAsync(m.cj, cj.data(), sizeof(CompactJob) * (size_t)B, cudaMemcpyHostToDevice, st));
-    if (int rc = launch_compact_edges(st, m.cj, B, maxC, false, true)) return rc;
+    if (int rc = launch_compact_edges(st, m.cj, B, maxC, false, true, narrow)) return rc;
     if (sharded) {
       std::vector<unsigned long long> off32(shard_off);
       for (auto& o : off32) o *= 2ull;
@@ -815,12 +817,11 @@
     const double elapsed =
         std::chrono::duration_cast<std::chrono::microseconds>(std::chrono::steady_clock::now() - t_begin).count() / 1e6;
     if (round_start_pending) {
-      engine_round_start_kernel<<<B, kCtlThreads, 0, st>>>(m.jobs, m.sl, m.sb, m.gj, m.cq, P, m.n_done);
-      PSU_CHECK_LAUNCH("engine_round_start_kernel");
-      if (int rc = launch_sample(st, m.sl, B, draws_bound, max_cap, true)) return rc;
+      if (int rc = launch_round_start(st, B, m.jobs, m.sl, m.sb, m.gj, m.cq, P, m.n_done, narrow)) return rc;
+      if (int rc = launch_sample(st, m.sl, B, draws_bound, max_cap, max_ccap, narrow)) return rc;
       launches += 5;
     }
-    if (int rc = launch_sample(st, m.sb, B, draws_bound, max_cap)) return rc;
+    if (int rc = launch_sample(st, m.sb, B, draws_bound, max_cap, 0, narrow)) return rc;
     if (ratio) {
       engine_scale_kernel<<<B, kCtlThreads, 0, st>>>(m.jobs, m.gj, m.cq, P);
       PSU_CHECK_LAUNCH("engine_scale_kernel");
diff --git a/probabilistic-self-update-line-vector-set-based-point-cloud-registration_b200/csrc/engine.cuh b/probabilistic-self-update-line-vector-set-based-point-cloud-registration_b200/csrc/engine.cuh
--- a/probabilistic-self-update-line-vector-set-based-point-cloud-registration_b200/csrc/engine.cuh
+++ b/probabilistic-self-update-line-vector-set-based-point-cloud-registration_b200/csrc/engine.cuh
@@ -8,6 +8,7 @@
 #include <vector>
 
 #include "common.cuh"
+#include "edge_fmt.cuh"
 
 namespace psulvsb {
 
@@ -42,7 +43,7 @@
   int n, stride;
   const uint32_t* row_counts;
   unsigned long long* offsets;
-  uint2* edges;
+  void* edges;
   unsigned long long cap;
   unsigned long long* n_edges;
   int active;
@@ -66,7 +67,7 @@
   unsigned int* class_counts;
   unsigned long long* class_offsets;
   unsigned long long* n_edges;
-  uint2* edges;
+  void* edges;
   unsigned long long cap;
   int* bad;
   int active;
@@ -88,7 +89,7 @@
   unsigned long long* status;
   int identity;
   int post;
-  const uint2* edges;
+  const void* edges;
   const uint32_t* via;
   uint2* gathered;
   const double* pts8;
@@ -158,10 +159,11 @@
 int launch_interleave_points(cudaStream_t st, const float4* in, int n, float4* out);
 int launch_consistency_mask(cudaStream_t st, const K1Job* d_jobs, int n_jobs, int max_n, int max_rows, bool row_sectors);
 int launch_symmetrize(cudaStream_t st, uint32_t* mask, int n, int stride);
-int launch_compact_edges(cudaStream_t st, const CompactJob* d_jobs, int n_jobs, int max_n, bool scan, bool emit);
+int launch_compact_edges(cudaStream_t st, const CompactJob* d_jobs, int n_jobs, int max_n, bool scan, bool emit,
+                         bool narrow);
 int ratio_count(cudaStream_t st, std::vector<RatioJob>& rj, RatioJob* d_rj, int max_n,
                 const std::function<void*(size_t)>& hist_arena, cudaEvent_t ev0, cudaEvent_t ev1);
-int ratio_emit(cudaStream_t st, const std::vector<RatioJob>& rj, RatioJob* d_rj, int max_n);
+int ratio_emit(cudaStream_t st, const std::vector<RatioJob>& rj, RatioJob* d_rj, int max_n, bool narrow);
 
 __host__ __device__ inline unsigned long long sample_max_draws_formula(unsigned long long n,
                                                                        unsigned long long count) {
@@ -186,7 +188,7 @@
 unsigned long long sample_list_counters();
 unsigned long long sample_table_words(unsigned long long n, unsigned long long max_draws);
 int launch_sample(cudaStream_t st, const SampleJob* d_jobs, int n_jobs, unsigned long long max_draws_bound,
-                  unsigned long long n_bound, bool flag_pass = false);
+                  unsigned long long n_bound, int flag_points = 0, bool narrow = false);
 int launch_philox_fill(cudaStream_t st, uint64_t seed, uint32_t domain, uint32_t event, unsigned long long first_k,
                        unsigned long long count, uint32_t* out);
 
diff --git a/probabilistic-self-update-line-vector-set-based-point-cloud-registration_b200/csrc/engine_kernels.cu b/probabilistic-self-update-line-vector-set-based-point-cloud-registration_b200/csrc/engine_kernels.cu
--- a/probabilistic-self-update-line-vector-set-based-point-cloud-registration_b200/csrc/engine_kernels.cu
+++ b/probabilistic-self-update-line-vector-set-based-point-cloud-registration_b200/csrc/engine_kernels.cu
@@ -216,6 +216,7 @@
   }
 }
 
+template <class F>
 __global__ void __launch_bounds__(BLK)
     engine_round_start_kernel(JobCtl* __restrict__ jobs, SampleJob* __restrict__ sl, SampleJob* __restrict__ sb,
                               GncJob* __restrict__ gj, CliqueJob* __restrict__ cq, EngineParams P,
@@ -277,7 +278,7 @@
       const int cnt = m0 + i;
       for (int j = tid; j < cnt; j += BLK) {
         const int other = (j < m0) ? J.inlier_map[j] : (C + (j - m0));
-        J.edges[off + j] = make_uint2((unsigned)(C + i), (unsigned)other);
+        F::store(J.edges, off + j, (unsigned)(C + i), (unsigned)other);
       }
     }
   }
@@ -332,6 +333,16 @@
   }
 }
 
+int launch_round_start(cudaStream_t st, int n_jobs, JobCtl* jobs, SampleJob* sl, SampleJob* sb, GncJob* gj, CliqueJob* cq,
+                       const EngineParams& P, int* n_done, bool narrow) {
+  if (narrow)
+    engine_round_start_kernel<EdgeNarrow><<<n_jobs, BLK, 0, st>>>(jobs, sl, sb, gj, cq, P, n_done);
+  else
+    engine_round_start_kernel<EdgeWide><<<n_jobs, BLK, 0, st>>>(jobs, sl, sb, gj, cq, P, n_done);
+  PSU_CHECK_LAUNCH("engine_round_start_kernel");
+  return PSULVSB_OK;
+}
+
 __global__ void __launch_bounds__(BLK)
     engine_scale_kernel(JobCtl* __restrict__ jobs, GncJob* __restrict__ gj, CliqueJob* __restrict__ cq, EngineParams P) {
   JobCtl& J = jobs[blockIdx.x];
diff --git a/probabilistic-self-update-line-vector-set-based-point-cloud-registration_b200/csrc/engine_kernels.cuh b/probabilistic-self-update-line-vector-set-based-point-cloud-registration_b200/csrc/engine_kernels.cuh
--- a/probabilistic-self-update-line-vector-set-based-point-cloud-registration_b200/csrc/engine_kernels.cuh
+++ b/probabilistic-self-update-line-vector-set-based-point-cloud-registration_b200/csrc/engine_kernels.cuh
@@ -9,8 +9,8 @@
 
 __global__ void engine_init_kernel(JobCtl* jobs, SampleJob* sl, SampleJob* sb, GncJob* gj, CliqueJob* cq,
                                    const unsigned long long* n_edges, EngineParams P, int* n_done);
-__global__ void engine_round_start_kernel(JobCtl* jobs, SampleJob* sl, SampleJob* sb, GncJob* gj, CliqueJob* cq,
-                                          EngineParams P, int* n_done);
+int launch_round_start(cudaStream_t st, int n_jobs, JobCtl* jobs, SampleJob* sl, SampleJob* sb, GncJob* gj, CliqueJob* cq,
+                       const EngineParams& P, int* n_done, bool narrow);
 __global__ void engine_scale_kernel(JobCtl* jobs, GncJob* gj, CliqueJob* cq, EngineParams P);
 __global__ void engine_local_control_kernel(JobCtl* jobs, SampleJob* sl, SampleJob* sb, GncJob* gj, CliqueJob* cq,
                                             EngineParams P, double elapsed_s, int* n_done);
diff --git a/probabilistic-self-update-line-vector-set-based-point-cloud-registration_b200/csrc/engine_state.cuh b/probabilistic-self-update-line-vector-set-based-point-cloud-registration_b200/csrc/engine_state.cuh
--- a/probabilistic-self-update-line-vector-set-based-point-cloud-registration_b200/csrc/engine_state.cuh
+++ b/probabilistic-self-update-line-vector-set-based-point-cloud-registration_b200/csrc/engine_state.cuh
@@ -64,7 +64,7 @@
   double* xs_sorted;
   uint8_t* sampled_flags;
   uint8_t* rot_flags;
-  uint2* edges;
+  void* edges;
   unsigned long long edge_cap;
   uint32_t* vbits;
   uint32_t* blist;
diff --git a/probabilistic-self-update-line-vector-set-based-point-cloud-registration_b200/csrc/k1_consistency.cu b/probabilistic-self-update-line-vector-set-based-point-cloud-registration_b200/csrc/k1_consistency.cu
--- a/probabilistic-self-update-line-vector-set-based-point-cloud-registration_b200/csrc/k1_consistency.cu
+++ b/probabilistic-self-update-line-vector-set-based-point-cloud-registration_b200/csrc/k1_consistency.cu
@@ -455,22 +455,27 @@
   }
 }
 
+template <class F>
 __global__ void compact_edges_kernel(const CompactJob* __restrict__ jobs) {
   const CompactJob& job = jobs[blockIdx.y];
   if (!job.active || !job.edges) return;
   const uint32_t* __restrict__ mask = job.mask;
   const int n = job.n, stride = job.stride;
   const unsigned long long cap = job.cap;
-  uint2* __restrict__ edges = job.edges;
+  void* __restrict__ edges = job.edges;
   const int row = (int)(((long long)blockIdx.x * blockDim.x + threadIdx.x) >> 5);
   const int lane = threadIdx.x & 31;
   if (row >= n) return;
-  if (job.row_counts && job.row_counts[row] == 0u) return;
+  const unsigned int count = job.row_counts ? job.row_counts[row] : 1u;
   const int W = (n + 31) >> 5;
   unsigned long long base = job.offsets[row];
+  const uint32_t* __restrict__ mrow = mask + (size_t)row * stride;
+  uint32_t next = (row >> 5) + lane < W ? mrow[(row >> 5) + lane] : 0u;
+  if (count == 0u) return;
   for (int w0 = row >> 5; w0 < W; w0 += 32) {
     const int w = w0 + lane;
-    uint32_t word = (w < W) ? mask[(size_t)row * stride + w] : 0u;
+    uint32_t word = next;
+    next = (w + 32 < W) ? mrow[w + 32] : 0u;
     const int pc = __popc(word);
     int incl = pc;
 #pragma unroll
@@ -482,7 +487,7 @@
     while (word) {
       const int b = __ffs(word) - 1;
       word &= word - 1;
-      if (pos < cap) edges[pos] = make_uint2((unsigned)row, (unsigned)(w * 32 + b));
+      if (pos < cap) F::store(edges, pos, (unsigned)row, (unsigned)(w * 32 + b));
       ++pos;
     }
     base += (unsigned long long)__shfl_sync(0xffffffffu, incl, 31);
@@ -583,7 +588,8 @@
   return PSULVSB_OK;
 }
 
-int launch_compact_edges(cudaStream_t st, const CompactJob* d_jobs, int n_jobs, int max_n, bool scan, bool emit) {
+int launch_compact_edges(cudaStream_t st, const CompactJob* d_jobs, int n_jobs, int max_n, bool scan, bool emit,
+                         bool narrow) {
   if (n_jobs <= 0 || max_n < 1) return PSULVSB_OK;
   if (scan) {
     row_scan_kernel<<<n_jobs, 1024, 0, st>>>(d_jobs);
@@ -592,7 +598,10 @@
   if (emit) {
     const long long threads = (long long)max_n * 32;
     dim3 grid((unsigned)((threads + 255) / 256), n_jobs);
-    compact_edges_kernel<<<grid, 256, 0, st>>>(d_jobs);
+    if (narrow)
+      compact_edges_kernel<EdgeNarrow><<<grid, 256, 0, st>>>(d_jobs);
+    else
+      compact_edges_kernel<EdgeWide><<<grid, 256, 0, st>>>(d_jobs);
     PSU_CHECK_LAUNCH("compact_edges_kernel");
   }
   return PSULVSB_OK;
diff --git a/probabilistic-self-update-line-vector-set-based-point-cloud-registration_b200/csrc/k1_ratio.cu b/probabilistic-self-update-line-vector-set-based-point-cloud-registration_b200/csrc/k1_ratio.cu
--- a/probabilistic-self-update-line-vector-set-based-point-cloud-registration_b200/csrc/k1_ratio.cu
+++ b/probabilistic-self-update-line-vector-set-based-point-cloud-registration_b200/csrc/k1_ratio.cu
@@ -301,6 +301,7 @@
   }
 }
 
+template <class F>
 __global__ void __launch_bounds__(256) ratio_class_emit_kernel(const RatioJob* __restrict__ jobs) {
   const RatioJob& job = jobs[blockIdx.y];
   if (!job.active || !job.edges) return;
@@ -322,7 +323,7 @@
       const unsigned int m = __ballot_sync(0xffffffffu, c == cc);
       if (c == cc) {
         const unsigned long long p = pos[cc] + (unsigned long long)__popc(m & ((1u << lane) - 1u));
-        if (p < job.cap) job.edges[p] = make_uint2((unsigned)row, (unsigned)(row + 1 + k));
+        if (p < job.cap) F::store(job.edges, p, (unsigned)row, (unsigned)(row + 1 + k));
       }
       pos[cc] += (unsigned long long)__popc(m);
     }
@@ -331,7 +332,8 @@
 
 }
 
-static int launch_ratio_reduced_set(cudaStream_t st, const RatioJob* d_jobs, int n_jobs, int max_n, int phase) {
+static int launch_ratio_reduced_set(cudaStream_t st, const RatioJob* d_jobs, int n_jobs, int max_n, int phase,
+                                    bool narrow = false) {
   if (n_jobs <= 0 || max_n < 2) return PSULVSB_OK;
   const long long row_threads = (long long)max_n * 32;
   const dim3 row_grid((unsigned)((row_threads + 255) / 256), (unsigned)n_jobs);
@@ -358,7 +360,10 @@
     ratio_class_scan_kernel<<<n_jobs, 1024, 0, st>>>(d_jobs);
     PSU_CHECK_LAUNCH("ratio_class_scan_kernel");
   } else {
-    ratio_class_emit_kernel<<<row_grid, 256, 0, st>>>(d_jobs);
+    if (narrow)
+      ratio_class_emit_kernel<EdgeNarrow><<<row_grid, 256, 0, st>>>(d_jobs);
+    else
+      ratio_class_emit_kernel<EdgeWide><<<row_grid, 256, 0, st>>>(d_jobs);
     PSU_CHECK_LAUNCH("ratio_class_emit_kernel");
   }
   return PSULVSB_OK;
@@ -405,9 +410,9 @@
   return PSULVSB_OK;
 }
 
-int ratio_emit(cudaStream_t st, const std::vector<RatioJob>& rj, RatioJob* d_rj, int max_n) {
+int ratio_emit(cudaStream_t st, const std::vector<RatioJob>& rj, RatioJob* d_rj, int max_n, bool narrow) {
   PSU_CUDA(cudaMemcpyAsync(d_rj, rj.data(), sizeof(RatioJob) * rj.size(), cudaMemcpyHostToDevice, st));
-  return launch_ratio_reduced_set(st, d_rj, (int)rj.size(), max_n, 2);
-}
-
-}
+  return launch_ratio_reduced_set(st, d_rj, (int)rj.size(), max_n, 2, narrow);
+}
+
+}
diff --git a/probabilistic-self-update-line-vector-set-based-point-cloud-registration_b200/csrc/k2_sampler.cu b/probabilistic-self-update-line-vector-set-based-point-cloud-registration_b200/csrc/k2_sampler.cu
--- a/probabilistic-self-update-line-vector-set-based-point-cloud-registration_b200/csrc/k2_sampler.cu
+++ b/probabilistic-self-update-line-vector-set-based-point-cloud-registration_b200/csrc/k2_sampler.cu
@@ -13,6 +13,8 @@
 constexpr int SMB_THREADS = 1024;
 constexpr int SMP_BW = 49152;
 constexpr int SMP_MAX_LIST_BUCKETS = 512;
+constexpr int SMF_THREADS = 256;
+constexpr int SMF_MAX_POINTS = 65536 * 8;
 
 struct ListPlan {
   unsigned int n_buckets, w_bits, width;
@@ -419,6 +421,7 @@
   if (tid == 0 && carry_s < job.count && job.status) job.status[0] = 0ull;
 }
 
+template <class F>
 __global__ void __launch_bounds__(SMP_THREADS) sample_emit_kernel(const SampleJob* __restrict__ jobs) {
   const SampleJob& job = jobs[blockIdx.y];
   if (!job.active) return;
@@ -431,11 +434,11 @@
          r += (unsigned long long)gridDim.x * SMP_THREADS) {
       out[r] = (uint32_t)r;
       if (job.post == 1) {
-        const uint2 e = job.edges[r];
+        const uint2 e = F::load(job.edges, r);
         job.flags[e.x] = 1;
         job.flags[e.y] = 1;
       } else if (job.post == 2) {
-        job.gathered[r] = job.edges[job.via[r]];
+        job.gathered[r] = F::load(job.edges, job.via[r]);
       }
     }
     if (blockIdx.x == 0 && tid == 0 && job.status) job.status[0] = 1ull;
@@ -484,11 +487,11 @@
             const uint32_t v = vv[l];
             out[rank] = v;
             if (job.post == 1 && !job.vbits) {
-              const uint2 e = job.edges[v];
+              const uint2 e = F::load(job.edges, v);
               job.flags[e.x] = 1;
               job.flags[e.y] = 1;
             } else if (job.post == 2) {
-              const uint2 e = job.edges[job.via[v]];
+              const uint2 e = F::load(job.edges, job.via[v]);
               job.gathered[rank] = e;
               if (job.lv_out && rank < job.lv_cap) {
                 const double2* pa = reinterpret_cast<const double2*>(job.pts8 + 8 * (size_t)e.x);
@@ -517,17 +520,35 @@
   }
 }
 
-__global__ void __launch_bounds__(256) sample_flag_kernel(const SampleJob* __restrict__ jobs) {
+template <class F>
+__global__ void __launch_bounds__(SMF_THREADS) sample_flag_kernel(const SampleJob* __restrict__ jobs, int onchip_points) {
   const SampleJob& job = jobs[blockIdx.y];
   if (!job.active || job.identity || job.post != 1 || !job.vbits) return;
+  extern __shared__ uint32_t pbits[];
+  const int tid = threadIdx.x;
+  const bool onchip = job.n_points <= onchip_points;
+  const int pwords = (job.n_points + 31) >> 5;
+  if (onchip) {
+    for (int i = tid; i < pwords; i += SMF_THREADS) pbits[i] = 0u;
+    __syncthreads();
+  }
+  uint8_t* __restrict__ flags = job.flags;
+  auto mark = [&](uint32_t p) {
+    if (!onchip) {
+      flags[p] = 1;
+      return;
+    }
+    const uint32_t bit = 1u << (p & 31u);
+    if (!(pbits[p >> 5] & bit)) atomicOr(&pbits[p >> 5], bit);
+  };
   const unsigned long long nwords = (job.n + 31) >> 5;
-  const unsigned long long threads = (unsigned long long)gridDim.x * 256;
-  const uint2* __restrict__ edges = job.edges;
-  for (unsigned long long wi = (unsigned long long)blockIdx.x * 256 + threadIdx.x; wi < nwords; wi += threads) {
+  const unsigned long long threads = (unsigned long long)gridDim.x * SMF_THREADS;
+  const void* __restrict__ edges = job.edges;
+  for (unsigned long long wi = (unsigned long long)blockIdx.x * SMF_THREADS + tid; wi < nwords; wi += threads) {
     uint32_t word = __ldcg(job.vbits + wi);
     if (!word) continue;
     job.vbits[wi] = 0u;
-    const uint2* __restrict__ row = edges + wi * 32;
+    const unsigned long long row = wi * 32;
     while (word) {
       uint2 e[4];
       int m = 0;
@@ -536,16 +557,42 @@
         if (word) {
           const int bit = __ffs(word) - 1;
           word &= word - 1;
-          e[j] = row[bit];
+          e[j] = F::load(edges, row + bit);
           m = j + 1;
         }
       }
 #pragma unroll
       for (int j = 0; j < 4; ++j)
         if (j < m) {
-          job.flags[e[j].x] = 1;
-          job.flags[e[j].y] = 1;
-        }
+          mark(e[j].x);
+          mark(e[j].y);
+        }
+    }
+  }
+  if (!onchip) return;
+  __syncthreads();
+  for (int w = tid; w < pwords; w += SMF_THREADS) {
+    const uint32_t bits = pbits[w];
+    if (!bits) continue;
+    uint8_t* __restrict__ f = flags + 32 * (size_t)w;
+#pragma unroll
+    for (int h = 0; h < 2; ++h) {
+      const uint32_t half = (bits >> (16 * h)) & 0xFFFFu;
+      if (half == 0xFFFFu) {
+        reinterpret_cast<uint4*>(f)[h] = make_uint4(0x01010101u, 0x01010101u, 0x01010101u, 0x01010101u);
+        continue;
+      }
+#pragma unroll
+      for (int q = 0; q < 4; ++q) {
+        const uint32_t nib = (half >> (4 * q)) & 0xFu;
+        uint8_t* __restrict__ g = f + 16 * h + 4 * q;
+        if (nib == 0xFu)
+          *reinterpret_cast<uint32_t*>(g) = 0x01010101u;
+        else
+#pragma unroll
+          for (int l = 0; l < 4; ++l)
+            if ((nib >> l) & 1u) g[l] = 1;
+      }
     }
   }
 }
@@ -577,12 +624,15 @@
 }
 
 int launch_sample(cudaStream_t st, const SampleJob* d_jobs, int n_jobs, unsigned long long max_draws_bound,
-                  unsigned long long n_bound, bool flag_pass) {
+                  unsigned long long n_bound, int flag_points, bool narrow) {
   if (n_jobs <= 0) return PSULVSB_OK;
   static bool attr_set = false;
   const size_t smem = (size_t)SMP_BW * 4 + (size_t)SMP_BW / 8;
+  const int fsmem_max = SMF_MAX_POINTS / 8;
   if (!attr_set) {
     PSU_CUDA(cudaFuncSetAttribute(sample_bucket_kernel, cudaFuncAttributeMaxDynamicSharedMemorySize, (int)smem));
+    PSU_CUDA(cudaFuncSetAttribute(sample_flag_kernel<EdgeWide>, cudaFuncAttributeMaxDynamicSharedMemorySize, fsmem_max));
+    PSU_CUDA(cudaFuncSetAttribute(sample_flag_kernel<EdgeNarrow>, cudaFuncAttributeMaxDynamicSharedMemorySize, fsmem_max));
     attr_set = true;
   }
   const unsigned long long nchunks = (max_draws_bound + SMP_CHUNK - 1) / SMP_CHUNK;
@@ -600,14 +650,22 @@
   if (bx < 1) bx = 1;
   sample_bucket_kernel<<<dim3((unsigned)bx, (unsigned)n_jobs), SMB_THREADS, smem, st>>>(d_jobs);
   PSU_CHECK_LAUNCH("sample_bucket_kernel");
-  sample_emit_kernel<<<dim3((unsigned)gx, (unsigned)n_jobs), SMP_THREADS, 0, st>>>(d_jobs);
+  if (narrow)
+    sample_emit_kernel<EdgeNarrow><<<dim3((unsigned)gx, (unsigned)n_jobs), SMP_THREADS, 0, st>>>(d_jobs);
+  else
+    sample_emit_kernel<EdgeWide><<<dim3((unsigned)gx, (unsigned)n_jobs), SMP_THREADS, 0, st>>>(d_jobs);
   PSU_CHECK_LAUNCH("sample_emit_kernel");
-  if (flag_pass) {
-    unsigned long long fx = (n_bound + 32ull * 256 - 1) / (32ull * 256);
+  if (flag_points > 0) {
+    unsigned long long fx = (n_bound + 32ull * SMF_THREADS - 1) / (32ull * SMF_THREADS);
     const unsigned long long fcap = ((unsigned long long)sm_count() * 16 + (unsigned long long)n_jobs - 1) / (unsigned long long)n_jobs;
     if (fx > fcap) fx = fcap;
     if (fx < 1) fx = 1;
-    sample_flag_kernel<<<dim3((unsigned)fx, (unsigned)n_jobs), 256, 0, st>>>(d_jobs);
+    const int onchip_points = flag_points <= SMF_MAX_POINTS ? flag_points : 0;
+    const size_t fsmem = (size_t)(onchip_points + 31) / 32 * 4;
+    if (narrow)
+      sample_flag_kernel<EdgeNarrow><<<dim3((unsigned)fx, (unsigned)n_jobs), SMF_THREADS, fsmem, st>>>(d_jobs, onchip_points);
+    else
+      sample_flag_kernel<EdgeWide><<<dim3((unsigned)fx, (unsigned)n_jobs), SMF_THREADS, fsmem, st>>>(d_jobs, onchip_points);
     PSU_CHECK_LAUNCH("sample_flag_kernel");
   }
   return PSULVSB_OK;
```

After: 16030 (median of 6 runs). +3.3%, better.
